# ConwayBeyond/Funscript-Flow

Measured on AMD Instinct MI355X. Metric: 1080p frame-pairs/sec, higher is better.
Workload: dtype f32

## Files before the change

### funscript_flow_amd/_capi.py

```python
import ctypes as C
import os
import sys

import numpy as np

_HERE = os.path.dirname(os.path.abspath(__file__))
LIB_PATH = os.path.join(_HERE, "csrc", "libffl_hip.so")

FFL_OK = 0
FFL_MAX_BATCH = 256
KERNEL_CLASSES = ["k_gray", "k_pyr_level", "k_polyexp", "k_frontend", "k_update_matrices", "k_blur_solve",
                  "k_pass1", "k_radial"]
FFL_PROFILE_ALL = 0xFF

FFL_MAX_CELLS = 64
CELL_DTYPE = np.dtype([(k, "<f8") for k in ("mean_u", "mean_v", "mean_mag", "var_mag")])
GRID_CENTRE_DTYPE = np.dtype([("cx", "<f8"), ("cy", "<f8"), ("total_var", "<f8"), ("cells", "<i4"), ("empty", "<i4")])
CENTERS = ("variance", "track")
FFL_MAX_TRACKS, FFL_MAX_TRACK_RADIUS = 8, 32
TRACK_ON_CUT = ("hold", "home")
TRACK_OK, TRACK_CUT, TRACK_LOST, TRACK_CLAMPED = 0, 1, 2, 4
TRACK_STATE_DTYPE = np.dtype([("x", "<f8"), ("y", "<f8"), ("home_x", "<f8"), ("home_y", "<f8"), ("steps", "<i8"),
                              ("lost_run", "<i4"), ("pad", "<i4")])
TRACK_DTYPE = np.dtype([("x", "<f8"), ("y", "<f8"), ("du", "<f8"), ("dv", "<f8"), ("sw", "<f8"), ("count", "<i4"), ("status", "<i4")])
# ... 605 lines not shown
    sw, sh = int(src_size[0]), int(src_size[1])
    win, b = (C.c_int * 4)(), C.c_size_t()
    code = layout if isinstance(layout, int) else yuv_layout(layout)
    info = source_info(rotate, mirror, yuv_range)
    geom = (int(resize[0]), int(resize[1]), int(crop[0]), int(crop[1]), int(out_size[0]), int(out_size[1]), win, C.byref(b))
    if depth == 8:
        rc = _src_call(load(), "ffl_frontend_yuv_window", info, sw, sh, code, int(sw if stride is None else stride), *geom)
    else:
        rc = _src_call(load(), "ffl_frontend_yuv16_window", info, sw, sh, code, int(2 * sw if stride is None else stride),
                       int(depth), *geom)
    _check(rc, exc=ValueError)
    return tuple(win), b.value


def _map_array(map, out_size, supersample):
    if supersample not in REMAP_SUPERSAMPLES or isinstance(supersample, bool):
        raise ValueError(f"supersample must be one of {REMAP_SUPERSAMPLES}, got {supersample!r}")
    m = np.asarray(map)
    want = (supersample * int(out_size[1]), supersample * int(out_size[0]), 2)
    if m.dtype != np.int32 or m.shape != want:
        raise ValueError(f"a source map for a {out_size[0]}x{out_size[1]} operand at supersample={supersample} is an int32 array of "
                         f"shape {want} holding (qx, qy) in 1/32 px, got {m.dtype} {m.shape}")
    return np.ascontiguousarray(m)


def remap_check(map, out_size, src_size, supersample=1, rotate=0, mirror=False, yuv_range="limited"):
    info = source_info(rotate, mirror, yuv_range)
    m = _map_array(map, out_size, supersample)
    up, st, valid = (C.c_int * 4)(), (C.c_int * 4)(), C.c_size_t()
    _check(load().ffl_remap_check(m.ctypes.data, int(out_size[0]), int(out_size[1]), int(supersample), int(src_size[0]),
                                  int(src_size[1]), C.byref(info) if info is not None else None, up, st, C.byref(valid)),
           exc=ValueError)
    return tuple(up), tuple(st), valid.value


def remap_bytes(out_size, supersample=1):
    return _sizes("ffl_remap_bytes", out_size[0], out_size[1], supersample)


class Remap:

    def __init__(self, id, src_size, supersample, window, valid):
        self.id, self.src_size, self.supersample, self.window, self.valid = id, tuple(src_size), supersample, window, valid

    def __repr__(self):
        return f"Remap(id={self.id}, src_size={self.src_size}, supersample={self.supersample}, window={self.window})"


_i, _u, _f, _pd, _sz, _u64, _vp, _str = C.c_int, C.c_uint, C.c_float, C.c_ssize_t, C.c_size_t, C.c_uint64, C.c_void_p, C.c_char_p
_ip, _i32p, _fp, _dp, _szp, _vpp = (C.POINTER(t) for t in (C.c_int, C.c_int32, C.c_float, C.c_double, C.c_size_t, C.c_void_p))
_P = C.POINTER
_ctx = _vp
_FRAMES = (_ctx, _i, _i, _vpp, _i, _i, _pd)
_DEVICE = (_ctx, _i, _i, _vp, _i)
_YUV_WIN = (_i, _i, _i, _pd)
_PAIRS = (_ctx, _i, _ip, _ip, _ip, _i)
_RADIAL = (_ctx, _i, _ip, _dp, _dp, _ip, _i, _dp)
_WINDOW = (_ctx, _i, _ip, _i, _i, _i, _f, _i)
_SRC = "_src"
SIGNATURES = {
    "ffl_device_count": (_i, ()),
    "ffl_create": (_i, (_i,) * 6 + (_vpp,)),
    "ffl_destroy": (None, (_ctx,)),
    "ffl_last_error": (_str, (_ctx,)),
    "ffl_device_mem_info": (_i, (_i, _szp, _szp)),
    "ffl_estimate_bytes": (_i, (_i,) * 5 + (_szp, _szp)),
    "ffl_upload_frame": (_i, (_ctx, _i, _vp, _i, _i, _i, _pd)),
    "ffl_upload_frames": (_i, (_ctx, _i, _i, _vpp, _i, _i, _i, _pd)),
    "ffl_upload_frames_raw": (_i, _FRAMES + (_i,) * 5),
    "ffl_upload_frames_raw_src": _SRC,
    "ffl_upload_frames_yuv": (_i, _FRAMES + (_i,) * 5),
    "ffl_frontend_yuv_window": (_i, _YUV_WIN + (_i,) * 6 + (_ip, _szp)),
    "ffl_upload_frames_yuv_src": _SRC,
    "ffl_frontend_yuv_window_src": _SRC,
    "ffl_upload_frames_yuv16": (_i, _FRAMES + (_i,) * 7),
    "ffl_frontend_yuv16_window": (_i, _YUV_WIN + (_i,) * 7 + (_ip, _szp)),
    "ffl_upload_frames_yuv16_src": _SRC,
    "ffl_frontend_yuv16_window_src": _SRC,
    "ffl_dev_frame_check": (_i, (_i,) * 3 + (_P(DevFrame),) + (_i,) * 6),
    "ffl_upload_frames_device": (_i, _DEVICE + (_i,) * 6 + (_u64,)),
    "ffl_dev_frame_check16": (_i, (_i,) * 4 + (_P(DevFrame),) + (_i,) * 6),
    "ffl_upload_frames_device16": (_i, _DEVICE + (_i,) * 8 + (_u64,)),
    "ffl_dev_frame_check_src": _SRC,
    "ffl_dev_frame_check16_src": _SRC,
    "ffl_upload_frames_device_src": _SRC,
    "ffl_upload_frames_device16_src": _SRC,
    "ffl_remap_check": (_i, (_vp,) + (_i,) * 5 + (_P(SourceInfo), _ip, _ip, _szp)),
    "ffl_remap_bytes": (_i, (_i,) * 3 + (_szp,)),
    "ffl_remap_create": (_i, (_ctx, _vp, _i, _i, _i, _ip)),
    "ffl_remap_destroy": (_i, (_ctx, _i)),
    "ffl_upload_frames_remap": (_i, (_ctx, _i, _i, _vpp, _i, _i, _i, _pd, _i, _i, _i, _P(SourceInfo))),
    "ffl_upload_frames_device_remap": (_i, _DEVICE + (_i,) * 5 + (_u64, _P(SourceInfo))),
    "ffl_export_flows": (_i, (_ctx, _i, _ip, _vp, _i, _pd, _u64)),
    "ffl_dev_flow_check": (_i, (_i,) * 4 + (_P(DevFlow),)),
    "ffl_import_flows": (_i, (_ctx, _i, _ip, _P(DevFlow), _i, _i, _u64)),
    "ffl_host_alloc": (_i, (_ctx, _sz, _vpp)),
    "ffl_host_free": (_i, (_ctx, _vp)),
    "ffl_flow_pairs": (_i, _PAIRS),
    "ffl_pass1_result": (_i, (_ctx, _i, _f, _i32p, _i32p, _fp, _fp, _ip)),
    "ffl_pass1_results": (_i, (_ctx, _i, _ip, _f, _i32p, _i32p, _fp, _fp, _ip)),
    "ffl_radial": (_i, _RADIAL),
    "ffl_radial_window": (_i, _WINDOW + (_vp, _u64)),
    "ffl_radial_axes": (_i, _RADIAL),
    "ffl_radial_window_axes": (_i, _WINDOW + (_vp, _u64)),
    "ffl_axes_extra_bytes": (_i, (_i, _i, _szp)),
    "ffl_dev_weights_check": (_i, (_i,) * 3 + (_P(DevWeights),)),
    "ffl_pass1_weighted": (_i, (_ctx, _i, _ip, _P(DevWeights), _i, _u64)),
    "ffl_radial_window_axes_weighted": (_i, _WINDOW + (_P(DevWeights), _vp, _u64)),
    "ffl_weights_extra_bytes": (_i, (_i, _i, _szp)),
    "ffl_consistency_default_params": (_i, (_P(ConsistencyParams),)),
    "ffl_consistency_params_check": (_i, (_P(ConsistencyParams),)),
    "ffl_consistency_weights": (_i, (_ctx, _i, _ip, _ip, _P(ConsistencyParams), _P(DevWeights), _P(DevWeights), _u64)),
    "ffl_residual_default_params": (_i, (_P(ResidualParams),)),
    "ffl_residual_params_check": (_i, (_P(ResidualParams),)),
    "ffl_residual_weights": (_i, (_ctx, _i, _ip, _ip, _ip, _P(ResidualParams), _P(DevWeights), _P(DevWeights), _u64)),
    "ffl_texture_default_params": (_i, (_P(TextureParams),)),
    "ffl_texture_params_check": (_i, (_P(TextureParams),)),
    "ffl_texture_weights": (_i, (_ctx, _i, _ip, _P(TextureParams), _P(DevWeights), _P(DevWeights), _u64)),
    "ffl_cell_grid_check": (_i, (_i,) * 3 + (_ip, _ip)),
    "ffl_cell_stats": (_i, (_ctx, _i, _ip, _i, _vp, _vp, _u64)),
    "ffl_radial_window_axes_centres": (_i, _WINDOW + (_vp, _pd, _vp, _u64)),
    "ffl_cells_extra_bytes": (_i, (_i,) * 3 + (_szp,)),
    "ffl_track_default_params": (_i, (_P(TrackParams),)),
    "ffl_track_params_check": (_i, (_P(TrackParams),)),
    "ffl_track_advance": (_i, (_ctx, _i, _ip, _i, _P(TrackParams), _P(DevWeights), _vp, _vp, _u64)),
    "ffl_roi_default_params": (_i, (_P(RoiParams),)),
    "ffl_roi_params_check": (_i, (_P(RoiParams),)),
    "ffl_roi_weights": (_i, (_ctx, _i, _vp, _pd, _P(RoiParams), _P(DevWeights), _P(DevWeights), _u64)),
    "ffl_radial_window_axes_weighted_centres": (_i, _WINDOW + (_P(DevWeights), _vp, _pd, _vp, _u64)),
    "ffl_motion_default_params": (_i, (_P(MotionParams),)),
    "ffl_motion_params_check": (_i, (_P(MotionParams),)),
    "ffl_motion_solve": (_i, (_dp, _i, _vp)),
    "ffl_motion_extra_bytes": (_i, (_i, _i, _szp)),
    "ffl_motion_fit": (_i, (_ctx, _i, _ip, _P(MotionParams), _P(DevWeights), _vp, _pd, _vp, _vp, _u64)),
    "ffl_motion_subtract": (_i, (_ctx, _i, _ip, _ip, _vp, _pd, _i, _u64)),
    "ffl_download_flow": (_i, (_ctx, _i, _vp)),
    "ffl_upload_flow": (_i, (_ctx, _i, _vp, _i)),
    "ffl_submit_pair": (_i, (_ctx, _i, _vp, _vp, _i, _i, _i, _pd, _i)),
    "ffl_sync": (_i, (_ctx,)),
    "ffl_dis_default_params": (_i, (_P(DisParams),)),
    "ffl_dis_geometry": (_i, (_i, _i, _P(DisParams), _ip, _ip)),
    "ffl_flow_pairs_dis": (_i, _PAIRS + (_P(DisParams),)),
    "ffl_debug_dis_pair": (_i, (_ctx, _i, _i, _P(DisParams), _i, _i, _vp)),
    "ffl_farneback_default_params": (_i, (_P(FarnebackParams),)),
    "ffl_farneback_geometry": (_i, (_i, _i, _P(FarnebackParams), _ip, _szp)),
    "ffl_farneback_extra_bytes": (_i, (_i,) * 3 + (_P(FarnebackParams), _szp)),
    "ffl_flow_pairs_farneback": (_i, _PAIRS + (_P(FarnebackParams),)),
    "ffl_flow_pairs_farneback_ex": (_i, _PAIRS + (_P(FarnebackParams), _u)),
    "ffl_num_levels": (_i, (_ctx,)),
    "ffl_level_size": (_i, (_ctx, _i, _ip)),
    "ffl_download_frame": (_i, (_ctx, _i, _vp)),
    "ffl_debug_pair": (_i, (_ctx,) + (_i,) * 4 + (_vp,) * 6),
    "ffl_debug_blur_plan": (_i, (_i,) * 9 + (_ip, _ip, _ip, _ip, _i)),
    "ffl_set_option": (_i, (_str, _i)),
    "ffl_ctx_set_option": (_i, (_ctx, _str, _i)),
    "ffl_ctx_get_option": (_i, (_ctx, _str, _ip)),
    "ffl_graph_stats": (_i, (_ctx, _ip, _ip, _ip)),
    "ffl_profile_enable": (_i, (_ctx, _u)),
    "ffl_profile_read": (_i, (_ctx, _i, _ip, _dp)),
    "ffl_kernel_name": (_str, (_i,)),
}
for _name, _sig in SIGNATURES.items():
    if _sig is _SRC:
        SIGNATURES[_name] = (SIGNATURES[_name[:-4]][0], SIGNATURES[_name[:-4]][1] + (_P(SourceInfo),))
EXPORTS = list(SIGNATURES)
RECORDS = {"ffl_source_info": SourceInfo, "ffl_dev_frame": DevFrame, "ffl_dev_flow": DevFlow, "ffl_pass2_record": PASS2_DTYPE,
           "ffl_axes_record": PASS2_AXES_DTYPE, "ffl_dev_weights": DevWeights, "ffl_consistency_params": ConsistencyParams,
           "ffl_residual_params": ResidualParams, "ffl_texture_params": TextureParams,
           "ffl_cell_record": CELL_DTYPE, "ffl_grid_centre": GRID_CENTRE_DTYPE, "ffl_motion_params": MotionParams,
           "ffl_motion_record": MOTION_DTYPE, "ffl_dis_params": DisParams, "ffl_track_params": TrackParams,
           "ffl_track_state": TRACK_STATE_DTYPE, "ffl_track_record": TRACK_DTYPE, "ffl_roi_params": RoiParams,
           "ffl_farneback_params": FarnebackParams}

_lib = None


def load():
    global _lib
    if _lib is not None:
        return _lib
    if not os.path.exists(LIB_PATH):
        raise FFLError(f"{LIB_PATH} is missing: build it with `make -C funscript_flow_amd/csrc` "
                       "(there is no CPU fallback for the HIP backend)")
    L = C.CDLL(LIB_PATH)
    for name, (restype, argtypes) in SIGNATURES.items():
        fn = getattr(L, name)
        fn.restype, fn.argtypes = restype, argtypes
    _lib = L
    return L


def set_option(name, value):
    if load().ffl_set_option(name.encode(), int(value)) != FFL_OK:
        raise FFLError(f"ffl_set_option({name!r}, {value}) rejected")


def get_option(name):
    v = C.c_int()
    if load().ffl_ctx_get_option(None, name.encode(), C.byref(v)) != FFL_OK:
        raise FFLError(f"unknown option {name!r}")
    return v.value


def blur_plan(tiles_x, tiles_y, n_pairs, slots, blur_rows=0, blur_min_wgs=3500, blur_taper=0, blur_taper_pairs=0,
              tile_order=0, blocks=True):
    L = load()
    args = [int(v) for v in (tiles_x, tiles_y, n_pairs, slots, blur_rows, blur_min_wgs, blur_taper, blur_taper_pairs, tile_order)]
    seg, n, grid = (C.c_int * 15)(), C.c_int(), C.c_int()
    _check(L.ffl_debug_blur_plan(*args, seg, C.byref(n), C.byref(grid), None, 0), exc=ValueError)
    segments = [tuple(seg[5 * i:5 * i + 5]) for i in range(n.value)]
    if not blocks:
        return segments, grid.value, None
    out = np.zeros((grid.value, 4), np.int32)
    _check(L.ffl_debug_blur_plan(*args, seg, C.byref(n), C.byref(grid), out.ctypes.data_as(_ip), grid.value), exc=ValueError)
    return segments, grid.value, out


def device_count():
    return load().ffl_device_count()


def device_mem_info(device=0):
    return _sizes("ffl_device_mem_info", device, outs=2)


def estimate_bytes(width, height, frame_slots, flow_slots, max_batch):
    return _sizes("ffl_estimate_bytes", width, height, frame_slots, flow_slots, max_batch, outs=2)


def axes_extra_bytes(width, height):
    return _sizes("ffl_axes_extra_bytes", width, height)


def weights_extra_bytes(width, height):
    return _sizes("ffl_weights_extra_bytes", width, height)


def cells_extra_bytes(width, height, cells):
    return _sizes("ffl_cells_extra_bytes", width, height, cells)


def motion_extra_bytes(width, height):
    return _sizes("ffl_motion_extra_bytes", width, height)


def cell_grid(width, height, cells):
    gw, gh = C.c_int(), C.c_int()
    _check(load().ffl_cell_grid_check(int(width), int(height), int(cells), C.byref(gw), C.byref(gh)))
    return gw.value, gh.value


def _centre_entries(centres, n_seq):
    if isinstance(centres, tuple) and len(centres) == 2 and isinstance(centres[1], (int, np.integer)):
        base, stride = centres
        return (int(base) if isinstance(base, (int, np.integer)) else _array_view(base)[0]), int(stride)
    ptr, shp, st, ts = _array_view(centres)
    if ts in ("<f8", "torch.float64") and len(shp) == 2:
        if shp != (n_seq, 2) or st[1] != 8:
            raise ValueError(f"centres: float64 shape {shp} with byte strides {st}, ({n_seq}, 2) with adjacent (cx, cy) is needed")
        return ptr, (st[0] if n_seq > 1 else 16)
    ptr, extent = _device_span(centres)
    if extent < n_seq * GRID_CENTRE_DTYPE.itemsize:
        raise ValueError(f"centres: {extent} bytes, {n_seq} centre records need {n_seq * GRID_CENTRE_DTYPE.itemsize}")
    return ptr, GRID_CENTRE_DTYPE.itemsize


def _iarr(v):
    a = np.ascontiguousarray(v, dtype=np.intc)
    return a.ctypes.data_as(C.POINTER(C.c_int)), a


def _darr(v):
    a = np.ascontiguousarray(v, dtype=np.float64)
    return a.ctypes.data_as(C.POINTER(C.c_double)), a


class Context:

    def __init__(self, width, height, device=0, frame_slots=None, flow_slots=None, max_batch=8):
        self.L = load()
        self.width, self.height, self.device, self.max_batch = int(width), int(height), int(device), int(max_batch)
        self.frame_slots = int(frame_slots if frame_slots is not None else 2 * max_batch + 2)
        self.flow_slots = int(flow_slots if flow_slots is not None else 13 + 2 * max_batch)
        h = C.c_void_p()
        rc = self.L.ffl_create(self.device, self.width, self.height, self.frame_slots, self.flow_slots, self.max_batch,
                               C.byref(h))
        if rc != FFL_OK:
            raise FFLError(f"ffl_create failed ({rc}): {self.L.ffl_last_error(None).decode()}")
        self._h = h

    def close(self):
        if getattr(self, "_h", None):
            self.L.ffl_destroy(self._h)
            self._h = None

    __del__ = close

    def __enter__(self):
        return self

    def __exit__(self, *a):
        self.close()

    def _chk(self, rc):
        if rc != FFL_OK:
            _check(rc, self._h)

    def upload_frame(self, fslot, frame):
        if frame.dtype != np.uint8 or frame.ndim not in (2, 3):
            raise FFLError("frame must be uint8 (H,W) or (H,W,3)")
        ch = 1 if frame.ndim == 2 else frame.shape[2]
        if frame.strides[-1] != 1 or (frame.ndim == 3 and frame.strides[1] != ch):
            frame = np.ascontiguousarray(frame)
        self._chk(self.L.ffl_upload_frame(self._h, fslot, frame.ctypes.data, frame.shape[1], frame.shape[0], ch,
                                          frame.strides[0]))

    def upload_frames(self, first_slot, frames):
        f0 = frames[0]
        shape, strides = f0.shape, f0.strides
        if f0.dtype == np.uint8 and f0.ndim in (2, 3) and strides[-1] == 1 and (f0.ndim == 2 or strides[1] == shape[2]):
            n = len(frames)
            ptrs = np.empty(n, np.uintp)
            uniform = True
            for i, f in enumerate(frames):
                if f.shape != shape or f.strides != strides or f.dtype != np.uint8:
                    uniform = False
                    break
                ptrs[i] = f.__array_interface__["data"][0]
            if uniform:
                ch = 1 if f0.ndim == 2 else shape[2]
                self._chk(self.L.ffl_upload_frames(self._h, first_slot, n, ptrs.ctypes.data_as(C.POINTER(C.c_void_p)), shape[1], shape[0],
                                                   ch, strides[0]))
                return
        fr = [f if (f.strides[-1] == 1 and (f.ndim == 2 or f.strides[1] == f.shape[2])) else np.ascontiguousarray(f)
              for f in frames]
        f0 = fr[0]
        ch = 1 if f0.ndim == 2 else f0.shape[2]
        if any(f.dtype != np.uint8 or f.shape != f0.shape or f.strides[0] != f0.strides[0] for f in fr):
            raise FFLError("upload_frames needs uint8 frames of one shape and row stride")
        ptrs = (C.c_void_p * len(fr))(*[f.ctypes.data for f in fr])
        self._chk(self.L.ffl_upload_frames(self._h, first_slot, len(fr), ptrs, f0.shape[1], f0.shape[0], ch,
                                           f0.strides[0]))

    def pinned_frames(self, n, channels=1, size=None, yuv=False, depth=8):
        w, h = size if size is not None else (self.width, self.height)
        shape = (n, h * 3 // 2, w) if yuv else (n, h, w) + ((channels,) if channels != 1 else ())
        dtype = np.uint8
        if depth != 8:
            if not yuv:
                raise FFLError("pinned_frames: depth applies to 4:2:0 frames (yuv=True)")
            dtype = np.uint16 if yuv_depth(depth)[0] > 8 else np.uint8
        nbytes = int(np.prod(shape)) * np.dtype(dtype).itemsize
        p = C.c_void_p()
        self._chk(self.L.ffl_host_alloc(self._h, nbytes, C.byref(p)))
        buf = (C.c_uint8 * nbytes).from_address(p.value)
        return np.frombuffer(buf, dtype).reshape(shape)

    def upload_frames_raw(self, first_slot, frames, resize, crop=(0, 0), rgb_order=False, rotate=0, mirror=False,
                          yuv_range="limited"):
        info = source_info(rotate, mirror, yuv_range)
        fr = [f if (f.ndim == 3 and f.strides[2] == 1 and f.strides[1] == 3) else np.ascontiguousarray(f) for f in frames]
        f0 = fr[0]
        if any(f.dtype != np.uint8 or f.ndim != 3 or f.shape != f0.shape or f.shape[2] != 3 or
               f.strides[0] != f0.strides[0] for f in fr):
            raise FFLError("upload_frames_raw needs (h, w, 3) uint8 frames of one shape and row stride")
        ptrs = (C.c_void_p * len(fr))(*[f.ctypes.data for f in fr])
        self._chk(_src_call(self.L, "ffl_upload_frames_raw", info, self._h, first_slot, len(fr), ptrs, f0.shape[1], f0.shape[0],
                            f0.strides[0], int(bool(rgb_order)), int(resize[0]), int(resize[1]), int(crop[0]), int(crop[1])))
# ... 456 lines not shown
```

### funscript_flow_amd/csrc/ffl_api.hip

```cpp
#include "../../include/ffl.h"
#include "ffl_kernels.h"

#include <math.h>
#include <stdarg.h>
#include <stdio.h>
#include <string.h>

#include <algorithm>
#include <condition_variable>
#include <mutex>
#include <string>
#include <thread>
#include <vector>

#define FFL_EV_RING 16
#define FFL_RAW_RING 4

template <class H, class Arg, hipError_t (*Free)(Arg)>
struct Owned {
    H h = H();
    Owned() = default;
    explicit Owned(H take) : h(take) {}
    Owned(Owned &&o) noexcept : h(o.release()) {}
    Owned &operator=(Owned &&o) noexcept { std::swap(h, o.h); return *this; }
// ... 262 lines not shown
};
typedef std::unique_lock<std::recursive_mutex> CtxLock;

static int set_err(ffl_ctx *c, int code, const char *fmt, ...) {
    char buf[512];
    va_list ap;
    va_start(ap, fmt);
    vsnprintf(buf, sizeof(buf), fmt, ap);
    va_end(ap);
    if (c) c->err = buf;
    else g_create_error = buf;
    return code;
}

#define HIPCHK_AS(c, what, call)                                                                          \
    do {                                                                                                  \
        hipError_t e_ = (call);                                                                           \
        if (e_ != hipSuccess)                                                                             \
            return set_err(c, FFL_ERR_HIP, "%s failed: %s (%s:%d)", what, hipGetErrorString(e_), __FILE__, \
                           __LINE__);                                                                     \
    } while (0)
#define HIPCHK(c, call) HIPCHK_AS(c, #call, call)
#define HIPCHK_ALLOC(c, fn, buf, ...) HIPCHK_AS(c, #fn "(" #buf ", " #__VA_ARGS__ ")", (buf).alloc(__VA_ARGS__))

static inline int cv_round(double v) { return (int)lrint(v); }

static void gaussian_kernel(int n, double sigma, float *out) {
    static const float tab1[] = {1.f};
    static const float tab3[] = {0.25f, 0.5f, 0.25f};
    static const float tab5[] = {0.0625f, 0.25f, 0.375f, 0.25f, 0.0625f};
    static const float tab7[] = {0.03125f, 0.109375f, 0.21875f, 0.28125f, 0.21875f, 0.109375f, 0.03125f};
    const float *fixed = nullptr;
    if (sigma <= 0 && (n & 1) && n <= 7) fixed = n == 1 ? tab1 : n == 3 ? tab3 : n == 5 ? tab5 : tab7;
    double sg = sigma > 0 ? sigma : ((n - 1) * 0.5 - 1) * 0.3 + 0.8;
    double scale2x = -0.5 / (sg * sg);
    double sum = 0;
    for (int i = 0; i < n; i++) {
        double x = i - (n - 1) * 0.5;
        double t = fixed ? (double)fixed[i] : exp(scale2x * x * x);
        out[i] = (float)t;
        sum += out[i];
    }
    sum = 1.0 / sum;
    for (int i = 0; i < n; i++) out[i] = (float)(out[i] * sum);
}

static void farneback_prepare_gaussian(int n, double sigma, FbgPoly *out) {
    float gg[2 * 7 + 1];
    double s = 0;
    for (int x = -n; x <= n; x++) {
        gg[x + n] = (float)exp(-x * x / (2 * sigma * sigma));
        s += gg[x + n];
    }
    s = 1. / s;
    for (int x = -n; x <= n; x++) gg[x + n] = (float)(gg[x + n] * s);
    for (int x = 0; x <= n; x++) {
        out->g[x] = gg[x + n];
        out->xg[x] = (float)(x * gg[x + n]);
        out->xxg[x] = (float)(x * x * gg[x + n]);
    }
    double G[6][6];
    memset(G, 0, sizeof(G));
    for (int y = -n; y <= n; y++)
        for (int x = -n; x <= n; x++) {
            float p = gg[y + n] * gg[x + n];
            G[0][0] += p;
            G[1][1] += p * x * x;
            G[3][3] += p * x * x * x * x;
            G[5][5] += p * x * x * y * y;
        }
    G[2][2] = G[0][3] = G[0][4] = G[3][0] = G[4][0] = G[1][1];
    G[4][4] = G[3][3];
    G[3][4] = G[4][3] = G[5][5];
    double A[6][12];
    for (int i = 0; i < 6; i++)
        for (int j = 0; j < 12; j++) A[i][j] = j < 6 ? G[i][j] : (j - 6 == i ? 1.0 : 0.0);
    for (int c = 0; c < 6; c++) {
        int p = c;
        for (int r = c + 1; r < 6; r++)
            if (fabs(A[r][c]) > fabs(A[p][c])) p = r;
        if (p != c)
            for (int j = 0; j < 12; j++) { double t = A[c][j]; A[c][j] = A[p][j]; A[p][j] = t; }
        double d = 1.0 / A[c][c];
        for (int j = 0; j < 12; j++) A[c][j] *= d;
        for (int r = 0; r < 6; r++)
            if (r != c) {
                double f = A[r][c];
                if (f != 0)
                    for (int j = 0; j < 12; j++) A[r][j] -= f * A[c][j];
            }
    }
    out->ig11 = A[1][7];
    out->ig03 = A[0][9];
    out->ig33 = A[3][9];
    out->ig55 = A[5][11];
}

static void polyexp_prepare(PolyConsts *pc) {
    FbgPoly q;
    farneback_prepare_gaussian(FFL_POLY_N, 1.2, &q);
    for (int x = 0; x <= FFL_POLY_N; x++) {
        pc->g[x] = q.g[x];
        pc->xg[x] = q.xg[x];
        pc->xxg[x] = q.xxg[x];
        pc->gd[x] = (double)pc->g[x];
        pc->xxgd[x] = (double)pc->xxg[x];
    }
    pc->ig11 = q.ig11;
    pc->ig03 = q.ig03;
    pc->ig33 = q.ig33;
    pc->ig55 = q.ig55;
}

struct LevelRule {
    int levels;
    int lw[FBG_MAX_SCALES], lh[FBG_MAX_SCALES], ksize[FBG_MAX_SCALES];
    double sigma[FBG_MAX_SCALES];
};
static void level_rule(int w, int h, double pyr_scale, int levels, LevelRule *r) {
    int k;
    double scale = 1.0;
    for (k = 0; k < levels; k++) {
        scale *= pyr_scale;
        if (w * scale < 32 || h * scale < 32) break;
    }
    r->levels = k;
    for (k = 0; k <= r->levels; k++) {
        double sc = 1.0;
        for (int i = 0; i < k; i++) sc *= pyr_scale;
        r->sigma[k] = (1.0 / sc - 1.0) * 0.5;
        const int sm = cv_round(r->sigma[k] * 5) | 1;
        r->ksize[k] = sm < 3 ? 3 : sm;
        r->lw[k] = cv_round(w * sc);
        r->lh[k] = cv_round(h * sc);
    }
}

static void level_geometry(int w, int h, Geometry *geo) {
    LevelRule r;
    level_rule(w, h, 0.5, 3, &r);
    geo->levels = r.levels;
    for (int k = 0; k <= r.levels; k++) {
        LevelGeom &g = geo->lv[k];
        g.lw = r.lw[k];
        g.lh = r.lh[k];
        g.ksize = r.ksize[k];
        g.sigma = r.sigma[k];
        memset(&g.gk, 0, sizeof(g.gk));
        g.gk.ksize = g.ksize;
        gaussian_kernel(g.ksize, g.sigma, g.gk.k);
    }
}

#define FFL_FRAME_SIZE_RULE "unsupported frame size %dx%d (16x16 .. 20*w*h < 2^32)"
static bool frame_size_ok(int w, int h) { return !(w < 16 || h < 16 || (long)w * h * 20 >= (1L << 32)); }
static bool counts_ok(int n_frame_slots, int n_flow_slots, int max_batch) {
    return n_frame_slots >= 2 && n_flow_slots >= 1 && max_batch >= 1 && max_batch <= FFL_MAX_BATCH;
}

static Layout context_layout(int w, int h, int n_frame_slots, int n_flow_slots, int max_batch) {
    Geometry geo;
    level_geometry(w, h, &geo);
    const size_t N = (size_t)w * h, maxU = 2 * (size_t)max_batch;
    Layout l = {};
    for (int k = 0; k <= geo.levels; k++) {
        const size_t plane = (size_t)geo.lv[k].lw * geo.lv[k].lh;
        l.i_off[k] = l.I; l.t_off[k] = l.T; l.r_off[k] = l.R;
        l.I += plane * maxU;
        l.T += ffl_pyr_tmp_floats(w, h, geo.lv[k].lw) * maxU;
        l.R += 5 * plane * maxU;
    }
    l.M = 5 * N * max_batch; l.flow = 2 * N * max_batch;
    l.p1 = (size_t)ffl_pass1_blocks(w, h) * max_batch; l.tab = FFL_EV_RING;
    l.gray = (size_t)n_frame_slots * N; l.bgr = (size_t)n_frame_slots * N * 3;
    l.slots = 2 * N * n_flow_slots; l.res = n_flow_slots;
    return l;
}

static hipEvent_t prof_event(ffl_ctx *c) {
    Event e;
    if (c->prof_pool.empty()) {
        hipEventCreate(e.put());
    } else {
        e = std::move(c->prof_pool.back());
        c->prof_pool.pop_back();
    }
    return e.release();
}

struct ProfScope {
    ffl_ctx *c;
    int cls;
    hipEvent_t a = nullptr, b = nullptr;
    bool on, shared = false;
    ProfScope(ffl_ctx *c_, int cls_, hipStream_t st, bool chain = false)
        : c(c_), cls(cls_), on((c_->prof_mask >> cls_) & 1u) {
        if (on) {
            stream = st;
            if (chain && c->prof_last_end && c->prof_last_cls == cls && c->prof_last_stream == st) {
                a = c->prof_last_end;
                shared = true;
            } else {
                a = prof_event(c);
                hipEventRecord(a, st);
            }
        } else {
            c->prof_last_end = nullptr;
        }
    }
    ~ProfScope() {
        if (on) {
            b = prof_event(c);
            hipEventRecord(b, stream);
            c->prof_recs.push_back({cls, a, b, shared});
            c->prof_last_end = b;
            c->prof_last_cls = cls;
            c->prof_last_stream = stream;
        }
    }
    hipStream_t stream = nullptr;
};

static void prof_collect(ffl_ctx *c) {
    for (auto &r : c->prof_recs) {
        float ms = 0;
        hipEventSynchronize(r.b);
        hipEventElapsedTime(&ms, r.a, r.b);
        c->prof_launches[r.cls]++;
        c->prof_ms[r.cls] += ms;
    }
    for (auto &r : c->prof_recs) {
        if (!r.shared_start) c->prof_pool.emplace_back(r.a);
        c->prof_pool.emplace_back(r.b);
    }
    c->prof_recs.clear();
    c->prof_last_end = nullptr;
}

struct WaitOnce {
    hipStream_t st;
    hipEvent_t seen[8];
    int n = 0;
    explicit WaitOnce(hipStream_t s) : st(s) {}
    hipError_t operator()(hipEvent_t e) {
        if (!e) return hipSuccess;
        for (int k = 0; k < n; k++)
            if (seen[k] == e) return hipSuccess;
        if (n < 8) seen[n++] = e;
        return hipStreamWaitEvent(st, e, 0);
    }
};

static int wait_unlocked(ffl_ctx *c, CtxLock &lk, const hipEvent_t *evs, int n) {
    HIPCHK(c, hipSetDevice(c->device));
    lk.unlock();
    hipError_t e = hipSuccess;
    for (int i = 0; i < n && e == hipSuccess; i++)
        if (evs[i]) e = hipEventSynchronize(evs[i]);
    lk.lock();
    if (e != hipSuccess) return set_err(c, FFL_ERR_HIP, "hipEventSynchronize failed: %s", hipGetErrorString(e));
    return FFL_OK;
}

static int wait_frame_free(ffl_ctx *c, WaitOnce &wait_copy, int fs) {
    const size_t nl = c->frame_readers();
    for (size_t l = 0; l < nl; l++) HIPCHK(c, wait_copy(c->ev_last_use[(size_t)fs * nl + l].get()));
    return FFL_OK;
}

static int publish_frames(ffl_ctx *c, int first, int n) {
    EvRef ev;
    HIPCHK(c, c->up_ring.record(c->s_copy, &ev));
    for (int i = first; i < first + n; i++) {
        c->ev_uploaded[i] = ev;
        c->frame_valid[i] = 1;
    }
    return FFL_OK;
}

static void publish_slots(ffl_ctx *c, int n, const int *slots, EvRef done, bool ready) {
    for (int i = 0; i < n; i++) {
        c->ev_slot_done[slots[i]] = done;
        c->slot_state[slots[i]] = ready;
    }
}

static int check_frame_run(ffl_ctx *c, const char *fn, int first, int n, const void *table, const uint8_t *const *frames = nullptr) {
    if (!table || n < 1 || first < 0 || first + n > c->n_fslots)
        return set_err(c, FFL_ERR_INVALID, "%s: bad frame slot range %d..%d", fn, first, first + n - 1);
    for (int i = 0; frames && i < n; i++)
        if (!frames[i]) return set_err(c, FFL_ERR_INVALID, "%s: frame %d is NULL", fn, i);
    return FFL_OK;
}

static bool flow_slot_ok(const ffl_ctx *c, int slot) { return slot >= 0 && slot < c->n_slots; }
static int check_flow_slots(ffl_ctx *c, const char *fn, int n, const int *slots, const char *holds, const char *repeat_rule) {
    for (int i = 0; i < n; i++) {
        if (!flow_slot_ok(c, slots[i])) return set_err(c, FFL_ERR_INVALID, "%s: flow slot %d out of range", fn, slots[i]);
        if (holds && !c->slot_state[slots[i]]) return set_err(c, FFL_ERR_STATE, "%s: flow slot %d holds no %s", fn, slots[i], holds);
    }
    if (!repeat_rule) return FFL_OK;
    int dup = -1;
    for (int i = 0; i < n; i++) {
        if (c->slot_mark[slots[i]] && dup < 0) dup = slots[i];
        c->slot_mark[slots[i]] = 1;
    }
// ... 561 lines not shown
                           crop_x, crop_y, out_w, out_h, win, bytes);
}

int ffl_frontend_yuv16_window_src(int src_w, int src_h, int layout, ptrdiff_t stride_bytes, int depth, int resize_w, int resize_h,
                                  int crop_x, int crop_y, int out_w, int out_h, int win[4], size_t *bytes,
                                  const ffl_source_info *si) {
    return frontend_window("ffl_frontend_yuv16_window", src_w, src_h, layout, stride_bytes, 2, depth, si, resize_w, resize_h,
                           crop_x, crop_y, out_w, out_h, win, bytes);
}

static int send_yuv(ffl_ctx *c, CtxLock &lk, const char *fn, int first, int n, const uint8_t *const *frames, int sw, int sh,
                    ptrdiff_t stride_bytes, int layout, int es, int depth, int msb, FrontParams &fp, const YuvWin &yw,
                    const RemapParams *rp) {
    for (int i = 0; es == 2 && i < n; i++)
        if ((uintptr_t)frames[i] & 1) return set_err(c, FFL_ERR_INVALID, "%s: frame %d is not 2-byte aligned", fn, i);
    HIPCHK(c, hipSetDevice(c->device));
    fp.kind = es == 2 ? FFL_SRC_YUV16 : FFL_SRC_YUV;
    fp.rgb = 0;
    if (es == 2) front_depth(&fp, depth, msb);
    const bool nv12 = layout == FFL_YUV_NV12;
    const size_t ybytes = (size_t)yw.w * yw.h * es, fbytes = ybytes * 3 / 2;
    struct Plane {
        size_t src, dst;
        ptrdiff_t pitch;
        size_t row;
        int rows;
    } pl[3];
    const size_t cw = (size_t)sw / 2 * es, ch = (size_t)sh / 2;
    const size_t wrow = (size_t)yw.w * es, x0 = (size_t)yw.x0 * es;
    pl[0] = {(size_t)yw.y0 * stride_bytes + x0, 0, stride_bytes, wrow, yw.h};
    int np = 3;
    if (nv12) {
        pl[1] = {(size_t)(sh + yw.y0 / 2) * stride_bytes + x0, ybytes, stride_bytes, wrow, yw.h / 2};
        np = 2;
    } else {
        const size_t u0 = (size_t)sh * sw * es + (size_t)(yw.y0 / 2) * cw + x0 / 2;
        pl[1] = {u0, ybytes, (ptrdiff_t)cw, wrow / 2, yw.h / 2};
        pl[2] = {u0 + ch * cw, ybytes + ybytes / 4, (ptrdiff_t)cw, wrow / 2, yw.h / 2};
    }
    const size_t span = (size_t)stride_bytes * (sh + sh / 2 - 1) + (size_t)sw * es;
    auto direct = [&](int i) {
        bool ok = in_host_buf(c, frames[i], span);
        for (int k = 0; ok && k < np; k++) ok = ((uintptr_t)(frames[i] + pl[k].src) | (size_t)pl[k].pitch | pl[k].row) % 4 == 0;
        return ok;
    };
    auto stage = [&](int i, uint8_t *h, int threads) {
        const uint8_t *src[2] = {frames[i] + pl[0].src, nullptr};
        c->pool.copy(h, src, 1, pl[0].pitch, pl[0].row, pl[0].rows, threads);
        src[0] = frames[i] + pl[1].src;
        if (!nv12) src[1] = frames[i] + pl[2].src;
        c->pool.copy(h + pl[1].dst, src, nv12 ? 1 : 2, pl[1].pitch, pl[1].row, pl[1].rows, threads);
    };
    auto send_direct = [&](int i, uint8_t *d) -> int {
        for (int k = 0; k < np; k++)
            HIPCHK(c, hipMemcpy2DAsync(d + pl[k].dst, pl[k].row, frames[i] + pl[k].src, (size_t)pl[k].pitch, pl[k].row,
                                       (size_t)pl[k].rows, hipMemcpyHostToDevice, c->s_copy));
        return FFL_OK;
    };
    auto desc = [&](const uint8_t *d) {
        FrameDesc s = {};
        s.p0 = d;
        s.p1 = d + ybytes;
        s.p2 = nv12 ? s.p1 + es : s.p1 + ybytes / 4;
        s.pitch0 = wrow;
        s.pitch1 = s.pitch2 = nv12 ? wrow : wrow / 2;
        s.c_step = (nv12 ? 2 : 1) * es;
        s.wx = yw.x0;
        s.wy = yw.y0;
        return s;
    };
    return upload_staged(c, lk, first, n, fbytes, fp, direct, stage, send_direct, desc, rp);
}

static int upload_yuv(ffl_ctx *c, const char *fn, int first, int n, const uint8_t *const *frames, int sw, int sh,
                      ptrdiff_t stride_bytes, int layout, int es, int depth, int msb, int rw, int rh, int crop_x, int crop_y,
                      const ffl_source_info *si) {
    if (!c) return FFL_ERR_INVALID;
    std::unique_lock<std::mutex> ul(c->up_mu);
    CtxLock lk(c->mu);
    if (int rc = check_frame_run(c, fn, first, n, frames, frames)) return rc;
    FrontParams fp;
    YuvWin yw;
    if (int rc = yuv_window(c, fn, sw, sh, layout, stride_bytes, es, depth, si, rw, rh, crop_x, crop_y, c->w, c->h, &fp, &yw))
        return rc;
    return send_yuv(c, lk, fn, first, n, frames, sw, sh, stride_bytes, layout, es, depth, msb, fp, yw, nullptr);
}

int ffl_upload_frames_yuv(ffl_ctx *c, int first, int n, const uint8_t *const *frames, int sw, int sh, ptrdiff_t stride_bytes,
                          int layout, int rw, int rh, int crop_x, int crop_y) {
    return upload_yuv(c, "ffl_upload_frames_yuv", first, n, frames, sw, sh, stride_bytes, layout, 1, 8, 0, rw, rh, crop_x, crop_y,
                      nullptr);
}

int ffl_upload_frames_yuv_src(ffl_ctx *c, int first, int n, const uint8_t *const *frames, int sw, int sh, ptrdiff_t stride_bytes,
                              int layout, int rw, int rh, int crop_x, int crop_y, const ffl_source_info *si) {
    return upload_yuv(c, "ffl_upload_frames_yuv", first, n, frames, sw, sh, stride_bytes, layout, 1, 8, 0, rw, rh, crop_x, crop_y, si);
}

int ffl_upload_frames_yuv16(ffl_ctx *c, int first, int n, const uint16_t *const *frames, int sw, int sh, ptrdiff_t stride_bytes,
                            int layout, int depth, int msb_aligned, int rw, int rh, int crop_x, int crop_y) {
    return upload_yuv(c, "ffl_upload_frames_yuv16", first, n, (const uint8_t *const *)frames, sw, sh, stride_bytes, layout, 2,
                      depth, msb_aligned != 0, rw, rh, crop_x, crop_y, nullptr);
}

int ffl_upload_frames_yuv16_src(ffl_ctx *c, int first, int n, const uint16_t *const *frames, int sw, int sh, ptrdiff_t stride_bytes,
                                int layout, int depth, int msb_aligned, int rw, int rh, int crop_x, int crop_y,
                                const ffl_source_info *si) {
    return upload_yuv(c, "ffl_upload_frames_yuv16", first, n, (const uint8_t *const *)frames, sw, sh, stride_bytes, layout, 2,
                      depth, msb_aligned != 0, rw, rh, crop_x, crop_y, si);
}

int ffl_upload_frame(ffl_ctx *c, int fslot, const uint8_t *data, int width, int height, int channels,
                     ptrdiff_t stride_bytes) {
    return ffl_upload_frames(c, fslot, 1, &data, width, height, channels, stride_bytes);
}

int ffl_download_frame(ffl_ctx *c, int fslot, uint8_t *dst) {
    if (!c) return FFL_ERR_INVALID;
    CtxLock lk(c->mu);
    if (!dst || fslot < 0 || fslot >= c->n_fslots)
        return set_err(c, FFL_ERR_INVALID, "ffl_download_frame: bad frame slot %d", fslot);
    if (!c->frame_valid[fslot]) return set_err(c, FFL_ERR_STATE, "ffl_download_frame: frame slot %d was never uploaded", fslot);
    HIPCHK(c, hipSetDevice(c->device));
    HIPCHK(c, hipMemcpyAsync(dst, c->d_gray + (size_t)fslot * c->N, c->N, hipMemcpyDeviceToHost, c->s_copy));
    HIPCHK(c, hipStreamSynchronize(c->s_copy));
    return FFL_OK;
}

struct DebugCapture {
    int level, iter;
    float *I0, *I1, *R0, *R1, *M, *flow;
};

static int enqueue_batch(ffl_ctx *c, ffl_ctx::Lane &L, const BatchTab &T, int n, int nU, int pov_mode, const DebugCapture *cap) {
    hipStream_t st = L.st;
    const size_t N = c->N;
    const UTab *ut = &L.d_tab->ut;
    const PairTab *pt = &L.d_tab->pt;
    const PyrJob *l0 = &L.pyr[L.n_jobs - 1];
    const bool fuse_l0 = c->opt.fuse_l0_blur && ffl_polyexp_from_gray_ok(*l0);
    const int skip_l0 = fuse_l0 && !cap;
    {
        ProfScope ps(c, FFL_K_PYRAMID, st);
        if (!ffl_launch_pyr_multi(c->d_gray, N, ut, nU, L.pyr, L.n_jobs - skip_l0, c->opt, st))
            for (int k = c->geo.levels; k >= skip_l0; k--)
                ffl_launch_pyr_level(c->d_gray, N, ut, nU, L.pyr[c->geo.levels - k], st);
    }
    {
        ProfScope ps(c, FFL_K_POLYEXP, st);
        ffl_launch_polyexp_multi(L.poly, L.n_jobs, nU, c->pc, c->d_gray, N, ut, fuse_l0 ? l0 : nullptr, st);
    }

    int pw = 0, ph = 0;
    for (int k = c->geo.levels; k >= 0; k--) {
        const LevelGeom &g = c->geo.lv[k];
        const int lw = g.lw, lh = g.lh;
        const size_t plane = (size_t)lw * lh;
        const size_t I_stride = plane, R_stride = 5 * plane, M_stride = 5 * plane;
        float *Rk = L.d_R + c->lay.r_off[k];
        if (pw == 0 && cap)
            for (int i = 0; i < n; i++) HIPCHK(c, hipMemsetAsync(T.pt.flow[k][i], 0, sizeof(float) * 2 * plane, st));
        int mi = 0;
        const bool fuse_first = c->opt.fuse_first > 0 && !cap && (long)((lw + 63) / 64) * ((lh + 15) / 16) * n >= c->opt.fuse_first;
        if (!fuse_first) {
            ProfScope ps(c, FFL_K_UPDATE_MATRICES, st);
            ffl_launch_update_matrices(Rk, R_stride, plane, pt, k, n, L.d_M[mi], M_stride, lw, lh, pw, ph, pw == 0, cap != nullptr, c->opt, st);
        }
        bool captured = false;
        auto capture = [&]() -> int {
            HIPCHK(c, hipStreamSynchronize(st));
            if (cap->I0) HIPCHK(c, hipMemcpy(cap->I0, L.d_I + c->lay.i_off[k] + (size_t)T.pt.u0[0] * I_stride, sizeof(float) * plane, hipMemcpyDeviceToHost));
            if (cap->I1) HIPCHK(c, hipMemcpy(cap->I1, L.d_I + c->lay.i_off[k] + (size_t)T.pt.u1[0] * I_stride, sizeof(float) * plane, hipMemcpyDeviceToHost));
            if (cap->R0) HIPCHK(c, hipMemcpy(cap->R0, Rk + (size_t)T.pt.u0[0] * R_stride, sizeof(float) * 5 * plane, hipMemcpyDeviceToHost));
            if (cap->R1) HIPCHK(c, hipMemcpy(cap->R1, Rk + (size_t)T.pt.u1[0] * R_stride, sizeof(float) * 5 * plane, hipMemcpyDeviceToHost));
            if (cap->M) HIPCHK(c, hipMemcpy(cap->M, L.d_M[mi], sizeof(float) * 5 * plane, hipMemcpyDeviceToHost));
            if (cap->flow) HIPCHK(c, hipMemcpy(cap->flow, T.pt.flow[k][0], sizeof(float) * 2 * plane, hipMemcpyDeviceToHost));
            captured = true;
            return FFL_OK;
        };
        for (int it = 0; it < 3; it++) {
            if (cap && cap->level == k && cap->iter == it) {
                int rc = capture();
                if (rc) return rc;
            }
            const int update = it < 2;
            {
                ProfScope ps(c, FFL_K_BLUR_SOLVE, st, it > 0 && !cap);
                if (it == 0 && fuse_first)
                    ffl_launch_blur_solve_first(L.d_M[mi ^ 1], M_stride, Rk, R_stride, plane, pt, k, n, lw, lh, pw, ph, c->opt, c->blur_slots, st);
                else
                    ffl_launch_blur_solve(L.d_M[mi], L.d_M[mi ^ 1], M_stride, Rk, R_stride, plane, pt, k, n, lw, lh,
                                          update, cap != nullptr, c->opt, c->blur_slots, st);
            }
            if (update) mi ^= 1;
        }
        if (cap && cap->level == k && !captured) {
            int rc = capture();
            if (rc) return rc;
        }
        pw = lw;
        ph = lh;
    }
    {
        ProfScope ps(c, FFL_K_PASS1, st);
        ffl_launch_pass1(pt, n, c->w, c->h, pov_mode, L.d_pkey, L.d_psum, st);
    }
    return FFL_OK;
}

static int batch_graph(ffl_ctx *c, ffl_ctx::Lane &L, const BatchTab &T, int n, int nU, int pov_mode,
                       ffl_ctx::Lane::GraphEntry **ge) {
    *ge = nullptr;
    for (auto &g : L.graphs)
        if (g.n == n && g.nU == nU && g.pov == pov_mode && g.epoch == c->opt_epoch) *ge = &g;
    if (*ge || c->graph_bad_epoch == c->opt_epoch) return FFL_OK;
    hipStream_t st = L.st;
    ffl_ctx::Lane::GraphEntry g = {n, nU, pov_mode, c->opt_epoch, Graph(), GraphExec()};
    hipError_t fail = hipStreamBeginCapture(st, hipStreamCaptureModeThreadLocal);
    if (fail == hipSuccess) {
        const int rc = enqueue_batch(c, L, T, n, nU, pov_mode, nullptr);
        fail = hipStreamEndCapture(st, g.graph.put());
        if (fail == hipSuccess && (rc != FFL_OK || !g.graph)) fail = hipErrorStreamCaptureInvalidated;
        if (fail == hipSuccess) fail = hipGraphInstantiate(g.exec.put(), g.graph, nullptr, nullptr, 0);
    }
    if (fail != hipSuccess) {
        g.exec.reset();
        g.graph.reset();
        (void)hipGetLastError();
        c->graph_bad_epoch = c->opt_epoch;
        c->graph_failed++;
        if (!c->graph_fail_reported) {
            c->graph_fail_reported = true;
            fprintf(stderr, "libffl_hip: hipGraph capture of a %d-pair batch failed (%s); this context launches its batches "
                            "one kernel at a time until its options change (results are unaffected)\n", n, hipGetErrorString(fail));
        }
        return FFL_OK;
    }
    if (L.graphs.size() >= 16) {
        HIPCHK(c, hipStreamSynchronize(st));
        L.graphs.erase(L.graphs.begin());
    }
    L.graphs.push_back(std::move(g));
    *ge = &L.graphs.back();
    c->graph_captured++;
    return FFL_OK;
}

static int fbg_work(ffl_ctx *c, ffl_ctx::Lane &L, const FbgPlan &p, int nU, FbgWork *wk);

static int queue_batch(ffl_ctx *c, ffl_ctx::Lane &L, BatchTab &T, int *nU_out, int n, const int *f0, const int *f1,
                       const int *slots, int pov_mode, const DebugCapture *cap, const DisKParams *dis,
                       const FbgPlan *fbg) {
    hipStream_t st = L.st;
    const size_t N = c->N;
    int nU = 0;
    auto uidx = [&](int fs) {
        int &u = c->u_of_fslot[fs];
        if (u < 0) {
            T.ut.fslot[nU] = fs;
            u = nU++;
        }
        return u;
    };
    for (int i = 0; i < n; i++) {
        T.pt.u0[i] = uidx(f0[i]);
        T.pt.u1[i] = uidx(f1[i]);
        T.pt.res[i] = c->d_res + slots[i];
    }
    for (int k = c->geo.levels; k >= 0; k--) {
        const size_t plane = (size_t)c->geo.lv[k].lw * c->geo.lv[k].lh;
        float *buf = ((c->geo.levels - k) & 1) ? L.d_flowB : L.d_flowA;
        for (int i = 0; i < n; i++)
            T.pt.flow[k][i] = (k == 0) ? c->d_flow + (size_t)slots[i] * 2 * N : buf + (size_t)i * 2 * plane;
    }
    for (int k = c->geo.levels + 1; k < FFL_MAX_LEVELS; k++)
        for (int i = 0; i < n; i++) T.pt.flow[k][i] = nullptr;
    for (int i = 0; i < nU; i++) c->u_of_fslot[T.ut.fslot[i]] = -1;
    *nU_out = nU;
    WaitOnce wait(st);
    for (int i = 0; i < nU; i++) HIPCHK(c, wait(c->ev_uploaded[T.ut.fslot[i]].get()));
    for (int i = 0; i < n; i++) HIPCHK(c, wait(c->ev_slot_done[slots[i]].get()));
    HIPCHK(c, hipMemcpyAsync(L.d_tab, &T, sizeof(BatchTab), hipMemcpyHostToDevice, st));

    if (fbg || dis) {
        if (fbg) {
            FbgWork wk;
            if (int rc = fbg_work(c, L, *fbg, nU, &wk)) return rc;
            ffl_launch_fb_general(&L.d_tab->ut, &L.d_tab->pt, n, nU, c->d_gray, N, c->w, c->h, *fbg, wk, st);
        } else {
            ffl_launch_dis(&L.d_tab->ut, &L.d_tab->pt, n, c->d_gray, N, L.d_M[0], *dis, st);
        }
        ProfScope ps(c, FFL_K_PASS1, st);
        ffl_launch_pass1(&L.d_tab->pt, n, c->w, c->h, pov_mode, L.d_pkey, L.d_psum, st);
    } else if (c->opt.use_graph && !cap && c->prof_mask == 0) {
        ffl_ctx::Lane::GraphEntry *ge;
        if (int rc = batch_graph(c, L, T, n, nU, pov_mode, &ge)) return rc;
        if (ge) {
            HIPCHK(c, hipGraphLaunch(ge->exec, st));
            c->graph_replayed++;
        } else if (int rc = enqueue_batch(c, L, T, n, nU, pov_mode, nullptr)) {
            return rc;
        }
    } else if (int rc = enqueue_batch(c, L, T, n, nU, pov_mode, cap)) {
        return rc;
    }
    HIPCHK(c, hipGetLastError());
    return FFL_OK;
// ... 1764 lines not shown
    *mode = (ps == 2 * e && cs == e && (e == 4 || al4)) ? FFL_IMP_NHWC : (e == 4 && ps == 4) ? FFL_IMP_NCHW : FFL_IMP_ANY;
    return FFL_OK;
}

int ffl_dev_flow_check(int dtype, int n, int width, int height, const ffl_dev_flow *f) {
    int mode;
    size_t bytes;
    return dev_flow_check(nullptr, "ffl_dev_flow_check", dtype, n, width, height, f, &mode, &bytes);
}

int ffl_import_flows(ffl_ctx *c, int n, const int *slots, const ffl_dev_flow *f, int dtype, int pov_mode, uint64_t stream) {
    static const char *fn = "ffl_import_flows";
    if (!c) return FFL_ERR_INVALID;
    std::unique_lock<std::mutex> pl(c->post_mu);
    CtxLock lk(c->mu);
    ExportTab t;
    if (int rc = open_slot_list(c, fn, "fields", n, slots, nullptr, &t)) return rc;
    int mode;
    size_t bytes;
    if (int rc = dev_flow_check(c, fn, dtype, n, c->w, c->h, f, &mode, &bytes)) return rc;
    hipStream_t cst;
    const PostRegion reg{"the flow fields", f->base, bytes, "host flow fields go through ffl_upload_flow"};
    if (int rc = post_begin(c, fn, stream, &cst, &reg, 1, n, slots)) return rc;
    const ImportArgs a{(const char *)f->base, (long long)f->item_stride, (long long)f->row_pitch, (long long)f->pixel_stride,
                       (long long)f->channel_stride, c->d_flow, c->d_res};
    {
        ProfScope ps(c, FFL_K_PASS1, c->s_post);
        ffl_launch_import_pass1(a, t, n, dtype, mode, c->w, c->h, pov_mode ? 1 : 0, c->d_ptab, c->d_pskey, c->d_rpsum,
                                c->s_post);
    }
    return post_end(c, cst, n, slots);
}

int ffl_upload_flow(ffl_ctx *c, int slot, const float *src, int pov_mode) {
    if (!c) return FFL_ERR_INVALID;
    std::unique_lock<std::mutex> pl(c->post_mu);
    CtxLock lk(c->mu);
    if (!flow_slot_ok(c, slot) || !src) return set_err(c, FFL_ERR_INVALID, "ffl_upload_flow: bad arguments");
    hipStream_t st = c->s_post;
    hipEvent_t ev = c->ev_slot_done[slot].get();
    if (int rc = wait_unlocked(c, lk, &ev, 1)) return rc;
    lk.unlock();
    hipError_t se = hipStreamSynchronize(st);
    lk.lock();
    HIPCHK(c, se);
    HIPCHK(c, hipMemcpy(c->d_flow + (size_t)slot * 2 * c->N, src, sizeof(float) * 2 * c->N, hipMemcpyHostToDevice));
    c->h_ptab->flow[0][0] = c->d_flow + (size_t)slot * 2 * c->N;
    c->h_ptab->res[0] = c->d_res + slot;
    HIPCHK(c, hipMemcpyAsync(c->d_ptab, c->h_ptab, sizeof(PairTab), hipMemcpyHostToDevice, st));
    {
        ProfScope ps(c, FFL_K_PASS1, st);
        ffl_launch_pass1(c->d_ptab, 1, c->w, c->h, pov_mode, c->d_pskey, c->d_rpsum, st);
    }
    EvRef done;
    if (int rc = publish_post(c, 1, &slot, &done)) return rc;
    HIPCHK(c, hipGetLastError());
    return FFL_OK;
}

int ffl_submit_pair(ffl_ctx *c, int slot, const uint8_t *prev, const uint8_t *next, int width, int height, int channels,
                    ptrdiff_t stride_bytes, int pov_mode) {
    if (!c) return FFL_ERR_INVALID;
    if (!flow_slot_ok(c, slot) || 2 * slot + 1 >= c->n_fslots) {
        CtxLock lk(c->mu);
        return set_err(c, FFL_ERR_INVALID, "ffl_submit_pair: slot %d needs frame slots %d,%d and a flow slot", slot, 2 * slot, 2 * slot + 1);
    }
    int rc = ffl_upload_frame(c, 2 * slot, prev, width, height, channels, stride_bytes);
    if (rc) return rc;
    rc = ffl_upload_frame(c, 2 * slot + 1, next, width, height, channels, stride_bytes);
    if (rc) return rc;
    int f0 = 2 * slot, f1 = 2 * slot + 1;
    return ffl_flow_pairs(c, 1, &f0, &f1, &slot, pov_mode);
}

int ffl_sync(ffl_ctx *c) {
    if (!c) return FFL_ERR_INVALID;
    std::unique_lock<std::mutex> ul(c->up_mu);
    std::unique_lock<std::mutex> pl(c->post_mu);
    CtxLock lk(c->mu);
    std::vector<hipEvent_t> evs;
    evs.push_back(ev_latest(c->up_ring).get());
    for (auto &rb : c->raw)
        if (rb.busy) evs.push_back(rb.ev);
    for (auto &L : c->lanes) evs.push_back(ev_latest(L.ring).get());
    evs.push_back(ev_latest(c->post_ring).get());
    pl.unlock();
    ul.unlock();
    return wait_unlocked(c, lk, evs.data(), (int)evs.size());
}

static constexpr struct { const char *name; int value; } kFixedKnobs[] = {
    {"blur_tile_h", 16}, {"run_ahead", 0}, {"merge_expand", 1}};
static const int *fixed_knob(const char *name) {
    for (const auto &k : kFixedKnobs)
        if (!strcmp(name, k.name)) return &k.value;
    return nullptr;
}
static const FflOptionRow *option_row(const char *name) {
    for (const FflOptionRow &r : kFflOptionRows)
        if (!strcmp(name, r.name)) return &r;
    return nullptr;
}

static int set_option_impl(FflOptions &o, const char *name, int value, bool live) {
    if (const int *fixed = fixed_knob(name)) return value == *fixed ? FFL_OK : FFL_ERR_INVALID;
    const FflOptionRow *r = option_row(name);
    if (!r || value < r->lo || value > r->hi) return FFL_ERR_INVALID;
    if (live && r->member == &FflOptions::lanes) return value == o.lanes ? FFL_OK : FFL_ERR_STATE;
    o.*r->member = r->flag ? value != 0 : value;
    return FFL_OK;
}

static int get_option_impl(const FflOptions &o, const char *name, int *value) {
    const int *fixed = fixed_knob(name);
    const FflOptionRow *r = option_row(name);
    if (!fixed && !r) return FFL_ERR_INVALID;
    *value = fixed ? *fixed : o.*r->member;
    return FFL_OK;
}

int ffl_debug_blur_plan(int tiles_x, int tiles_y, int n_pairs, int slots, int blur_rows, int blur_min_wgs, int blur_taper,
                        int blur_taper_pairs, int tile_order, int *segments, int *n_segments, int *grid, int *blocks,
                        int max_blocks) {
    FflOptions o;
    if (tiles_x < 1 || tiles_y < 1 || n_pairs < 1 || n_pairs > FFL_MAXB || slots < 0 || !segments || !n_segments || !grid ||
        set_option_impl(o, "blur_rows", blur_rows, false) || set_option_impl(o, "blur_min_wgs", blur_min_wgs, false) ||
        set_option_impl(o, "blur_taper", blur_taper, false) || set_option_impl(o, "blur_taper_pairs", blur_taper_pairs, false) ||
        set_option_impl(o, "tile_order", tile_order, false))
        return set_err(nullptr, FFL_ERR_INVALID, "ffl_debug_blur_plan: bad size, pair count, slot count, option value or NULL output");
    BlurPlan plan;
    const unsigned g = ffl_blur_plan(tiles_x, tiles_y, n_pairs, slots, o, &plan);
    *n_segments = plan.n;
    *grid = (int)g;
    for (int i = 0; i < FFL_BLUR_SEGS; i++) {
        const BlurSeg &s = plan.s[i];
        const int row[5] = {s.first_block, s.first_pair, s.pairs, s.nrb, s.strips};
        memcpy(segments + 5 * i, row, sizeof(row));
    }
    if (!blocks) return FFL_OK;
    if ((unsigned)max_blocks < g)
        return set_err(nullptr, FFL_ERR_INVALID, "ffl_debug_blur_plan: %u workgroups, room for %d", g, max_blocks);
    for (unsigned blk = 0; blk < g; blk++) {
        int b, tile_x, row0, nrb;
        int *out = blocks + 4 * (size_t)blk;
        if (ffl_blur_block(plan, blk, tiles_x, tile_order, b, tile_x, row0, nrb)) {
            out[0] = b; out[1] = tile_x; out[2] = row0; out[3] = std::max(0, std::min(nrb, tiles_y - row0));
        } else {
            out[0] = -1; out[1] = out[2] = out[3] = 0;
        }
    }
    return FFL_OK;
}

int ffl_set_option(const char *name, int value) {
    if (!name) return FFL_ERR_INVALID;
    std::lock_guard<std::mutex> g(g_opt_mu);
    return set_option_impl(g_opts, name, value, false);
}

int ffl_ctx_set_option(ffl_ctx *c, const char *name, int value) {
    if (!c || !name) return FFL_ERR_INVALID;
    CtxLock lk(c->mu);
    const int rc = set_option_impl(c->opt, name, value, true);
    if (rc == FFL_OK) c->opt_epoch++;
    else if (rc == FFL_ERR_STATE) set_err(c, rc, "ffl_ctx_set_option: \"lanes\" is fixed once the context exists (%d)", c->opt.lanes);
    else set_err(c, rc, "ffl_ctx_set_option: unknown option or value out of range: %s = %d", name, value);
    return rc;
}

int ffl_ctx_get_option(ffl_ctx *c, const char *name, int *value) {
    if (!name || !value) return FFL_ERR_INVALID;
    if (!c) {
        std::lock_guard<std::mutex> g(g_opt_mu);
        return get_option_impl(g_opts, name, value);
    }
    CtxLock lk(c->mu);
    return get_option_impl(c->opt, name, value);
}

int ffl_graph_stats(ffl_ctx *c, int *captured, int *replayed, int *capture_failures) {
    if (!c) return FFL_ERR_INVALID;
    CtxLock lk(c->mu);
    if (captured) *captured = c->graph_captured;
    if (replayed) *replayed = c->graph_replayed;
    if (capture_failures) *capture_failures = c->graph_failed;
    return FFL_OK;
}

int ffl_profile_enable(ffl_ctx *c, unsigned class_mask) {
    if (!c) return FFL_ERR_INVALID;
    int rc = ffl_sync(c);
    if (rc) return rc;
    CtxLock lk(c->mu);
    prof_collect(c);
    c->prof_mask = class_mask;
    return FFL_OK;
}

int ffl_profile_read(ffl_ctx *c, int k, int *launches, double *total_ms) {
    if (!c || k < 0 || k >= FFL_K_COUNT) return FFL_ERR_INVALID;
    int rc = ffl_sync(c);
    if (rc) return rc;
    CtxLock lk(c->mu);
    prof_collect(c);
    if (launches) *launches = c->prof_launches[k];
    if (total_ms) *total_ms = c->prof_ms[k];
    c->prof_launches[k] = 0;
    c->prof_ms[k] = 0;
    return FFL_OK;
}

}
```

### funscript_flow_amd/csrc/ffl_kernels.h

```cpp
#pragma once
#include <hip/hip_runtime.h>
#include <limits.h>
#include <stdint.h>

#define FFL_MAXB 256
#define FFL_MAXU (2 * FFL_MAXB)
#define FFL_MAX_LEVELS 4
#define FFL_POLY_N 5
#define FFL_WIN 15
#define FFL_WIN_R 7

struct PolyConsts {
    float g[FFL_POLY_N + 1], xg[FFL_POLY_N + 1], xxg[FFL_POLY_N + 1];
    double gd[FFL_POLY_N + 1], xxgd[FFL_POLY_N + 1];
    double ig11, ig03, ig33, ig55;
};

struct GaussKernel {
    float k[32];
    int ksize;
};

struct UTab {
    int fslot[FFL_MAXU];
};

struct PairTab {
    int u0[FFL_MAXB], u1[FFL_MAXB];
    float *flow[FFL_MAX_LEVELS][FFL_MAXB];
    struct Pass1Result *res[FFL_MAXB];
};

struct BatchTab {
    UTab ut;
    PairTab pt;
};

struct Pass1Result {
    int x, y;
    float div_val;
    int weighted;
    double mag_sum;
};
__host__ __device__ inline double ffl_record_mean(const Pass1Result &r, double npx) {
    return r.weighted ? r.mag_sum : r.mag_sum / npx;
}

enum { FFL_FRONT_GENERIC = 0, FFL_FRONT_AREA2 = 1, FFL_FRONT_IDENTITY = 2 };
enum { FFL_SRC_GRAY = 0, FFL_SRC_BGR = 1, FFL_SRC_YUV = 2, FFL_SRC_YUV16 = 3, FFL_SRC_ANY = -1 };
struct FrameDesc {
    const uint8_t *p0, *p1, *p2;
    long long pitch0, pitch1, pitch2;
    long long ps, cs;
    int c_step;
    int wx, wy;
    int fslot;
};
struct FrontParams {
    int kind, rgb;
    int sw, sh;
    int cx, cy, ow, oh;
    double scale_x, scale_y;
    int mode;
    int shift16, round16;
    int src;
    int ax, bx, cx0, ay, by, cy0;
    int full;
};
#define FFL_REMAP_NONE (-2147483647 - 1)
struct RemapParams {
    const int2 *map;
    int ss, lg;
};
struct ExportTab {
    int slot[FFL_MAXB];
};

enum { FFL_IMP_F32 = 0, FFL_IMP_F16 = 1, FFL_IMP_BF16 = 2 };
enum { FFL_IMP_ANY = 0,
       FFL_IMP_NHWC = 1,
       FFL_IMP_NCHW = 2 };
struct ImportArgs {
    const char *base;
    long long item, pitch, ps, cs;
    float *flow;
    Pass1Result *res;
};

struct WeightArgs {
    const char *base;
    long long item, pitch;
};

#define FFL_MAX_JOBS 4
enum { FFL_PYR_NONE = -1, FFL_PYR_F1 = 0, FFL_PYR_F2, FFL_PYR_H4, FFL_PYR_H9, FFL_PYR_V4, FFL_PYR_V9, FFL_PYR_H1 };
struct PyrJob {
    int kind, w, h, lw, lh;
    unsigned gx, gy, first, count;
    double sx, sy;
    float *tmp, *I;
    size_t tmp_stride, I_stride;
    GaussKernel gk;
};
struct PyrJobs {
    PyrJob j[FFL_MAX_JOBS];
    int n;
};
struct PolyJob {
    const float *I;
    float *R;
    size_t I_stride, R_stride, plane;
    int w, h;
    unsigned gx, gy, first, count;
    int from_gray;
    float gk0, gk1;
};
struct PolyJobs {
    PolyJob j[FFL_MAX_JOBS];
    int n;
};

struct FflOptions {
    int lanes = 2;
    int fuse_first = 10000;
    int use_graph = 1;
    int copy_threads = 4;
    int blur_rows = 0;
    int blur_min_wgs = 3500;
    int tile_order = 0;
    int blur_taper = 1;
    int blur_taper_pairs = 0;
    int pyr_coarse = 1;
    int fuse_l0_blur = 1;
    int fb_general = 0;
};
struct FflOptionRow {
    const char *name;
    int FflOptions::*member;
    int lo, hi;
    bool flag;
};
inline constexpr FflOptionRow kFflOptionRows[] = {
    {"lanes", &FflOptions::lanes, 1, 4, false},
    {"fuse_first", &FflOptions::fuse_first, 0, INT_MAX, false},
    {"graph", &FflOptions::use_graph, INT_MIN, INT_MAX, true},
    {"copy_threads", &FflOptions::copy_threads, 1, 16, false},
    {"blur_rows", &FflOptions::blur_rows, 0, 64, false},
    {"blur_min_wgs", &FflOptions::blur_min_wgs, 1, INT_MAX, false},
    {"tile_order", &FflOptions::tile_order, 0, 1, false},
    {"blur_taper", &FflOptions::blur_taper, 0, 1, false},
    {"blur_taper_pairs", &FflOptions::blur_taper_pairs, 0, FFL_MAXB, false},
    {"pyr_coarse", &FflOptions::pyr_coarse, INT_MIN, INT_MAX, true},
    {"fuse_l0_blur", &FflOptions::fuse_l0_blur, INT_MIN, INT_MAX, true},
    {"fb_general", &FflOptions::fb_general, 0, 1, false},
};

#define FFL_BLUR_SEGS 3
struct BlurSeg {
    int first_block, first_pair, pairs, nrb, strips;
};
struct BlurPlan {
    BlurSeg s[FFL_BLUR_SEGS];
    int n;
};
struct BlurSlots {
    int first, first_zero, update, last;
};

bool ffl_launch_pyr_multi(const uint8_t *gray_base, size_t gray_stride, const UTab *ut, int nU, const PyrJob *levels, int n,
                          const FflOptions &opt, hipStream_t st);
bool ffl_polyexp_from_gray_ok(const PyrJob &l0);
void ffl_launch_polyexp_multi(const PolyJob *levels, int n, int nU, PolyConsts pc, const uint8_t *gray_base, size_t gray_stride,
                              const UTab *ut, const PyrJob *l0, hipStream_t st);
void ffl_launch_frontend(const FrameDesc &d, uint8_t *gray, const FrontParams &p, hipStream_t st);
void ffl_launch_frontend_dev(const FrameDesc *tab, int n, uint8_t *gray_base, size_t N, const FrontParams &p, hipStream_t st);
void ffl_launch_frontend_remap(const FrameDesc &d, uint8_t *gray, const FrontParams &p, const RemapParams &r, hipStream_t st);
void ffl_launch_frontend_remap_dev(const FrameDesc *tab, int n, uint8_t *gray_base, size_t N, const FrontParams &p,
                                   const RemapParams &r, hipStream_t st);
void ffl_launch_export_flows(const float *flow, const ExportTab &tab, int n, size_t N, char *dst, long long item_stride,
                             int layout, hipStream_t st);
void ffl_launch_import_pass1(const ImportArgs &a, const ExportTab &tab, int n, int dtype, int mode, int w, int h, int pov_mode,
                             PairTab *pt, unsigned long long *pkey, double *psum, hipStream_t st);
void ffl_launch_gray(const uint8_t *bgr, uint8_t *gray, int n_pixels, hipStream_t st);
size_t ffl_pyr_tmp_floats(int w, int h, int lw);
bool ffl_pyr_level_ok(int w, int h, int lw, int lh, int ksize);
void ffl_launch_pyr_level(const uint8_t *gray_base, size_t gray_stride, const UTab *ut, int nU, const PyrJob &level,
                          hipStream_t st);
void ffl_launch_update_matrices(const float *R, size_t R_stride, size_t plane, const PairTab *pt, int level, int nB, float *M,
                                size_t M_stride, int lw, int lh, int pw, int ph, int zero_flow, int store_flow,
                                const FflOptions &opt, hipStream_t st);
void ffl_launch_blur_solve(const float *Min, float *Mout, size_t M_stride, const float *R, size_t R_stride,
                           size_t plane, const PairTab *pt, int level, int nB, int lw, int lh, int update, int store_flow,
                           const FflOptions &opt, const BlurSlots &slots, hipStream_t st);


void ffl_launch_blur_solve_first(float *Mout, size_t M_stride, const float *R, size_t R_stride, size_t plane,
                                 const PairTab *pt, int level, int nB, int lw, int lh, int pw, int ph, const FflOptions &opt,
                                 const BlurSlots &slots, hipStream_t st);
bool ffl_blur_slots(BlurSlots *out);
unsigned ffl_blur_plan(int tiles_x, int tiles_y, int nB, int slots, const FflOptions &opt, BlurPlan *plan);

#define DIS_MAX_PATCHES 4096
#define DIS_MAX_SCALES 12
struct DisKParams {
    int w, h, finest, coarsest, stride, gd_iters, vr_iters, mean_norm, spatial_prop, stripes;
    float alpha, gamma, delta;
    size_t pair_floats;
    size_t pyr_floats;
    size_t pyr_off[DIS_MAX_SCALES];
    float *dbg;
    int dbg_scale, dbg_stage;
};
void ffl_launch_dis(const UTab *ut, const PairTab *pt, int nB, const uint8_t *gray, size_t gray_stride, float *scratch,
                    const DisKParams &p, hipStream_t st);

int ffl_pass1_blocks(int w, int h);
void ffl_launch_pass1(const PairTab *pt, int nB, int w, int h, int pov_mode, unsigned long long *pkey, double *psum,
                      hipStream_t st);

#define FFL_WINDOW_MAX_RADIUS 32
struct WindowSeq {
    int slot[FFL_MAXB + 2 * FFL_WINDOW_MAX_RADIUS];
};
struct WindowItem {
    const float *flow;
    double cx, cy;
    int cut, pad;
};
struct Pass2Record {
    double dot, cx, cy;
    float mean_mag, div_val;
    int x, y, cut, pad;
};
struct AxesRecord {
    Pass2Record base;
    double tangential, shift_x, shift_y, reserved;
};
#define FFL_NAXES 4
int ffl_radial_blocks(int w, int h);
struct RadialForm {
    int nc;
    const WeightArgs *maps;
};
void ffl_launch_radial(const WindowItem *tab, int n, int w, int h, int pov_mode, const double *wytab, const RadialForm &form,
                       double *psum, void *out, hipStream_t st);
void ffl_launch_pass1_weighted(const WeightArgs &wa, float *flow, Pass1Result *res, const ExportTab &tab, int n, int w, int h,
                               int pov_mode, PairTab *pt, unsigned long long *pkey, double *psum, double *psw, hipStream_t st);
void ffl_launch_window_plan(const WindowSeq &seq, int n_seq, int first, int n, int radius, float cut_threshold,
                            const Pass1Result *res, const float *flow, int w, int h, const void *cen, long long cstride,
                            WindowItem *tab, void *out, int rec_stride, hipStream_t st);

#define FFL_CELLS_MAX 64
struct CellRecord {
    double mean_u, mean_v, mean_mag, var_mag;
};
struct GridCentre {
    double cx, cy, total_var;
    int cells, empty;
};
void ffl_launch_cell_stats(const float *flow, const ExportTab &tab, int n, int w, int h, int G, CellRecord *cells,
                           GridCentre *centres, double *rowsum, hipStream_t st);

void ffl_launch_consistency(const float *flow, const ExportTab &fwd, const ExportTab &bwd, int n, int w, int h, float alpha,
                            float beta, int soft, const WeightArgs *gate, char *out, long long out_item, long long out_pitch,
                            hipStream_t st);

void ffl_launch_residual(const unsigned char *gray, const float *flow, const ExportTab &fr0, const ExportTab &fr1, const ExportTab &fl,
                         int n, int w, int h, float alpha, float beta, int soft, const WeightArgs *gate, char *out,
                         long long out_item, long long out_pitch, hipStream_t st);

void ffl_launch_texture(const unsigned char *gray, const ExportTab &fr, int n, int w, int h, int radius, float tau, int soft,
                        const WeightArgs *gate, char *out, long long out_item, long long out_pitch, hipStream_t st);

#define FFL_TRACK_MAX_R 32
#define FFL_TRACK_MAX_T 8
enum { TRK_HOLD = 0, TRK_HOME = 1 };
enum { TRK_OK = 0, TRK_CUT = 1, TRK_LOST = 2, TRK_CLAMPED = 4 };
struct TrackState {
    double x, y, home_x, home_y;
    long long steps;
    int lost_run, pad;
};
struct TrackRecord {
    double x, y, du, dv, sw;
    int count, status;
};
void ffl_launch_track(const float *flow, const Pass1Result *res, const ExportTab &tab, int n, int n_tracks, int w, int h,
                      int radius, int on_cut, float cut_threshold, const WeightArgs *maps, TrackState *state, TrackRecord *out,
                      hipStream_t st);
void ffl_launch_roi_weights(const char *cen, long long cstride, int n, int w, int h, float ax, float ay, int soft,
                            const WeightArgs *gate, char *out, long long out_item, long long out_pitch, hipStream_t st);

#define FFL_MOTION_NSUMS 12
enum { MOT_S = 0, MOT_SX, MOT_SY, MOT_SXX, MOT_SXY, MOT_SYY, MOT_SU, MOT_SUX, MOT_SUY, MOT_SV, MOT_SVX, MOT_SVY };
enum { MOT_TRANSLATION = 0, MOT_RIGID = 1, MOT_SIMILARITY = 2, MOT_AFFINE = 3 };
enum { MOT_OK = 0, MOT_EMPTY = 1, MOT_DEGENERATE = 2 };
struct MotionRecord {
    double a0, a1, a2, b0, b1, b2;
    double sw;
    int model, status;
};
struct MotionPrior {
    const char *base;
    long long stride;
};

__host__ __device__ inline void ffl_motion_solve_body(const double *s, int model, MotionRecord *out) {
    const double S = s[MOT_S], Sx = s[MOT_SX], Sy = s[MOT_SY], Sxx = s[MOT_SXX], Sxy = s[MOT_SXY], Syy = s[MOT_SYY];
    const double Su = s[MOT_SU], Sux = s[MOT_SUX], Suy = s[MOT_SUY], Sv = s[MOT_SV], Svx = s[MOT_SVX], Svy = s[MOT_SVY];
    MotionRecord r;
    r.a0 = r.a1 = r.a2 = r.b0 = r.b1 = r.b2 = 0.0;
    r.sw = S;
    r.model = model;
    r.status = MOT_EMPTY;
    if (S == 0.0) {
        *out = r;
        return;
    }
    const double ta = Su / S, tb = Sv / S;
    r.a0 = ta;
    r.b0 = tb;
    r.status = MOT_OK;
    const double eps = 1e-12;
    if (model == MOT_RIGID || model == MOT_SIMILARITY) {
        const double Q = Sxx + Syy;
        const double q = Sx / S, p = Sy / S;
        const double D = (Q - q * Sx) - p * Sy;
        if (!(S > eps * S) || !(D > eps * Q)) {
            r.status = MOT_DEGENERATE;
        } else {
            const double g3 = Svx - Suy;
            const double z3 = (g3 + p * Su) - q * Sv;
            const double rot = z3 / D;
            double sc = 0.0;
            if (model == MOT_SIMILARITY) {
                const double g2 = Sux + Svy;
                const double z2 = (g2 - q * Su) - p * Sv;
                sc = z2 / D;
            }
            r.a0 = (ta - q * sc) + p * rot;
            r.b0 = (tb - p * sc) - q * rot;
            r.a1 = sc;
            r.a2 = -rot;
            r.b1 = rot;
            r.b2 = sc;
        }
    } else if (model == MOT_AFFINE) {
        bool ok = S > eps * S;
        double l10 = 0.0, l20 = 0.0, l21 = 0.0, d1 = 0.0, d2 = 0.0;
        if (ok) {
            l10 = Sx / S;
// ... 225 lines not shown
```

### funscript_flow_amd/csrc/kernels_farneback.hip

```cpp
#include "ffl_kernels.h"

#include <algorithm>

__global__ __launch_bounds__(256) void k_gray(const uint8_t *__restrict__ bgr, uint8_t *__restrict__ gray, int n) {
    int i4 = (blockIdx.x * 256 + threadIdx.x) * 4;
    if (i4 + 3 < n) {
        const uint32_t *p = reinterpret_cast<const uint32_t *>(bgr + (size_t)i4 * 3);
        uint32_t a = p[0], b = p[1], c = p[2];
        uint32_t px[12] = {a & 255, (a >> 8) & 255, (a >> 16) & 255, a >> 24, b & 255, (b >> 8) & 255,
                           (b >> 16) & 255, b >> 24, c & 255, (c >> 8) & 255, (c >> 16) & 255, c >> 24};
        uint32_t o = 0;
#pragma unroll
        for (int j = 0; j < 4; j++) {
            uint32_t g = (px[j * 3] * 3735u + px[j * 3 + 1] * 19235u + px[j * 3 + 2] * 9798u + 16384u) >> 15;
            o |= g << (8 * j);
        }
        *reinterpret_cast<uint32_t *>(gray + i4) = o;
    } else {
        for (int i = i4; i < n; i++) {
            uint32_t b = bgr[(size_t)i * 3], g = bgr[(size_t)i * 3 + 1], r = bgr[(size_t)i * 3 + 2];
            gray[i] = (uint8_t)((b * 3735u + g * 19235u + r * 9798u + 16384u) >> 15);
        }
    }
}
// ... 783 lines not shown
        ffl_um_finish(cur.r0, bb, cur.inside, w, h, x, y, cur.f.x, cur.f.y, m);
        if (in) {
#pragma unroll
            for (int c = 0; c < 5; c++) *ffl_at<float>(M + c * plane, o) = m[c];
        }
        if (k + 1 < NR) cur = nxt;
    }
}

template <int MODE>
__global__ __launch_bounds__(256) void k_update_matrices(const float *__restrict__ R, size_t R_stride, size_t plane,
                                                         const PairTab *__restrict__ pt, int level,
                                                         float *__restrict__ M, size_t M_stride, int w,
                                                         int h, int pw, int ph, double usx, double usy, int store_flow,
                                                         int nB, int order) {
    int b, tile_x, tile_y;
    if (!ffl_tile_coord((w + 63) / 64, (h + 15) / 16, nB, order, b, tile_x, tile_y)) return;
    const int lx = threadIdx.x & 63, x0 = tile_x * 64, x = min(x0 + lx, w - 1);
    const bool xin = x0 + lx < w;
    const float *R0 = R + (size_t)pt->u0[b] * R_stride, *R1 = R + (size_t)pt->u1[b] * R_stride;
    float *flow = pt->flow[level][b];
    const float *pf = pt->flow[min(level + 1, FFL_MAX_LEVELS - 1)][b];
    constexpr int NR = 4;
    const int ybase = tile_y * 16 + (threadIdx.x >> 6);
    float2 f[NR];
    if (MODE == 1) {
        const bool half_scale = usx == 0.5 && usy == 0.5;
        int xa0, xa1;
        float a1;
        if (half_scale) ffl_resize_coord_half(x, pw, xa0, xa1, a1);
        else ffl_resize_coord(x, pw, usx, xa0, xa1, a1);
        const int xq = min(xa0, pw - 2);
        float4 c0[NR], c1[NR];
        float b1[NR];
#pragma unroll
        for (int k = 0; k < NR; k++) {
            int ya0, ya1;
            const int y = min(ybase + 4 * k, h - 1);
            if (half_scale) ffl_resize_coord_half(y, ph, ya0, ya1, b1[k]);
            else ffl_resize_coord(y, ph, usy, ya0, ya1, b1[k]);
            c0[k] = ffl_gload4(pf, 8u * ((unsigned)ya0 * (unsigned)pw + xq));
            c1[k] = ffl_gload4(pf, 8u * ((unsigned)ya1 * (unsigned)pw + xq));
        }
#pragma unroll
        for (int k = 0; k < NR; k++) f[k] = ffl_upsample2(c0[k], c1[k], xa0 == xq, xa1 == xq, a1, b1[k]);
    } else if (MODE == 0) {
#pragma unroll
        for (int k = 0; k < NR; k++) {
            const unsigned o = (unsigned)min(ybase + 4 * k, h - 1) * (unsigned)w + (unsigned)x;
            const FFL_GLOBAL float *q = (const FFL_GLOBAL float *)flow + 2u * o;
            f[k] = make_float2(q[0], q[1]);
        }
    } else {
#pragma unroll
        for (int k = 0; k < NR; k++) f[k] = make_float2(0.f, 0.f);
    }
    ffl_um_rows<NR>(R0, R1, M + (size_t)b * M_stride, plane, w, h, x, xin, ybase, [&](int k) { return f[k]; },
                    [&](unsigned o, float2 d) {
                        if (MODE == 1 && store_flow) {
                            flow[2u * o] = d.x;
                            flow[2u * o + 1u] = d.y;
                        }
                    });
}

void ffl_launch_update_matrices(const float *R, size_t R_stride, size_t plane, const PairTab *pt, int level, int nB,
                                float *M,
                                size_t M_stride, int lw, int lh, int pw, int ph, int zero_flow, int store_flow,
                                const FflOptions &opt, hipStream_t st) {
    dim3 grid(ffl_tile_grid((lw + 63) / 64, (lh + 15) / 16, nB));
    const auto k = pw > 0 ? k_update_matrices<1> : (zero_flow ? k_update_matrices<2> : k_update_matrices<0>);
    hipLaunchKernelGGL(k, grid, dim3(256), 0, st, R, R_stride, plane, pt, level, M, M_stride, lw, lh, pw, ph,
                       pw > 0 ? (double)pw / lw : 1.0, pw > 0 ? (double)ph / lh : 1.0, pw > 0 ? store_flow : 0, nB,
                       opt.tile_order);
}

#ifndef FFL_K5_WAVES
#define FFL_K5_WAVES 4
#endif
#ifndef FFL_K5_WAVES_FIRST
#define FFL_K5_WAVES_FIRST 3
#endif
#ifndef FFL_K5_GROUP_FIRST
#define FFL_K5_GROUP_FIRST 3
#endif
#ifndef FFL_K5_GROUP
#define FFL_K5_GROUP 3
#endif

__device__ __forceinline__ void ffl_box_block16(const float (&v)[30], double (&out)[16]) {
    double s[15];
    s[14] = (double)v[14];
#pragma unroll
    for (int j = 13; j >= 0; j--) s[j] = (double)v[j] + s[j + 1];
    double p = (double)v[15];
    out[0] = s[0];
#pragma unroll
    for (int t = 1; t < 15; t++) {
        out[t] = s[t] + p;
        p = p + (double)v[15 + t];
    }
    out[15] = p;
}

template <int Q>
__device__ __forceinline__ void ffl_box_quarter(const double (&d)[18], double (&out)[4]) {
    constexpr int NA = 15 - 4 * Q;
    double S[4] = {0.0, 0.0, 0.0, 0.0};
    double s = d[NA - 1];
    if (NA - 1 < 4) S[NA - 1] = s;
#pragma unroll
    for (int j = NA - 2; j >= 0; j--) {
        s = d[j] + s;
        if (j < 4) S[j] = s;
    }
    double p = d[NA];
#pragma unroll
    for (int m = 0; m <= 4 * Q + 2; m++) {
        if (m > 0) p = p + d[NA + m];
        const int i = m + 1 - 4 * Q;
        if (i >= 0 && i < 4) {
            if (4 * Q + i == 15) out[i] = p;
            else out[i] = S[i] + p;
        }
    }
    if (Q == 0) out[0] = S[0];
}

#ifdef FFL_STAMP
#define FFL_NSTAMP 16
__device__ unsigned long long g_stamp[64][FFL_NSTAMP];
extern "C" int ffl_debug_read_stamps(unsigned long long *out) {
    return (int)hipMemcpyFromSymbol(out, HIP_SYMBOL(g_stamp), sizeof(unsigned long long) * 64 * FFL_NSTAMP);
}
#define FFL_DRAIN_MAX 8192
__device__ unsigned long long g_drain[3][FFL_DRAIN_MAX][2];
extern "C" int ffl_debug_read_drain(unsigned long long *out) {
    return (int)hipMemcpyFromSymbol(out, HIP_SYMBOL(g_drain), sizeof(unsigned long long) * 3 * FFL_DRAIN_MAX * 2);
}
#define FFL_DRAIN(e)                                                          \
    if (w >= 1024 && tid == 0 && blockIdx.x < FFL_DRAIN_MAX) g_drain[FIRST ? 0 : UPDATE ? 1 : 2][blockIdx.x][e] = wall_clock64();
#define FFL_T(i)                                                              \
    if (FFL_STAMP_ON && tid == 0) {                                           \
        const unsigned long long t_ = __builtin_readcyclecounter();          \
        sStamp[i] += t_ - sStamp[FFL_NSTAMP];                                 \
        sStamp[FFL_NSTAMP] = t_;                                              \
    }
#else
#define FFL_T(i)
#define FFL_DRAIN(e)
#endif


template <bool UPDATE, int FIRST>
__global__ __launch_bounds__(256, FIRST ? FFL_K5_WAVES_FIRST : FFL_K5_WAVES) void k_blur_solve(
    const float *__restrict__ Min, float *__restrict__ Mout, size_t M_stride, const float *__restrict__ R, size_t R_stride,
    size_t plane, const PairTab *__restrict__ pt, int level, int w, int h, BlurPlan plan, int pw, int ph, double usx, double usy,
    int store_flow, int order) {
    constexpr int TW = 64, TH = 16, LW = TW + 2 * FFL_WIN_R, LH = TH + 2 * FFL_WIN_R;
    constexpr int PX = 4;
    constexpr int NCARRY = LH - TH;
    constexpr int LW2 = 44;
    constexpr int GC = FIRST ? FFL_K5_GROUP_FIRST : FFL_K5_GROUP, NG = (5 + GC - 1) / GC;
    __shared__ double2 sS2[GC][TH][LW2];
    const int tid = threadIdx.x;
#ifdef FFL_STAMP
    __shared__ unsigned long long sStamp[FFL_NSTAMP + 1];
    const bool FFL_STAMP_ON = FIRST == 1 && w >= 1024;
    if (FFL_STAMP_ON && tid == 0) {
        for (int i = 0; i < FFL_NSTAMP; i++) sStamp[i] = 0;
        sStamp[FFL_NSTAMP] = __builtin_readcyclecounter();
    }
#endif
    int b, tile_x, row0, nrb;
    if (!ffl_blur_block(plan, blockIdx.x, (w + TW - 1) / TW, order, b, tile_x, row0, nrb)) return;
    FFL_DRAIN(0)
    const int x0 = tile_x * TW;
    const float *Mb = Min + (size_t)b * M_stride;

    const int q = __builtin_amdgcn_readfirstlane(tid >> 6);
    const int ty = (tid & 63) >> 2, kk = tid & 3;
    const int lx0 = 16 * kk + 4 * q;
    double *sS = reinterpret_cast<double *>(&sS2[0][0][0]);
    const int vcc = tid / LW, vtx = tid - vcc * LW;
    const int vgx = min(max(x0 + vtx - FFL_WIN_R, 0), w - 1);
    const unsigned pitch = (unsigned)w * 4u;
    float carry[NG][NCARRY];
    const double scale = 1.0 / (FFL_WIN * FFL_WIN);
    float2 *flow = reinterpret_cast<float2 *>(pt->flow[level][b]);
    const float *R0 = R + (size_t)pt->u0[b] * R_stride, *R1 = R + (size_t)pt->u1[b] * R_stride;
    float *Mo = Mout + (size_t)b * M_stride;
    constexpr int FP = TW + 2;
    float4 *sF4 = reinterpret_cast<float4 *>(&sS2[0][0][0]);
    constexpr int UP = 80;
    __shared__ float sM34[FIRST ? 5 - GC : 1][FIRST ? TH : 1][FIRST ? UP : 1];
    float *sM012 = reinterpret_cast<float *>(&sS2[0][0][0]);
    static_assert(GC * TH * UP * 4 <= (int)sizeof(sS2), "the first group's staged rows must fit the column sums");
    const float2 *prevf = reinterpret_cast<const float2 *>(pt->flow[min(level + 1, FFL_MAX_LEVELS - 1)][b]);
    struct UStageA {
        float a1, b1;
        float4 c0, c1;
        bool first0, first1;
        int r, tx, gx, gy;
    };
    const bool half_scale = usx == 0.5 && usy == 0.5;
    auto phase_u = [&](int y0, int jbase, int nrows) {
        const int N = LW * nrows;
        auto coords = [&](int i, int &r, int &tx, int &gx, int &gy) {
            r = i / LW;
            tx = i - r * LW;
            gy = min(max(y0 - FFL_WIN_R + jbase + r, 0), h - 1);
            gx = min(max(x0 + tx - FFL_WIN_R, 0), w - 1);
        };
        auto issue = [&](int i) {
            UStageA A;
            coords(i, A.r, A.tx, A.gx, A.gy);
            const int gx = A.gx, gy = A.gy;
            if (FIRST == 1) {
                int xa0, xa1, ya0, ya1;
                if (half_scale) {
                    ffl_resize_coord_half(gx, pw, xa0, xa1, A.a1);
                    ffl_resize_coord_half(gy, ph, ya0, ya1, A.b1);
                } else {
                    ffl_resize_coord(gx, pw, usx, xa0, xa1, A.a1);
                    ffl_resize_coord(gy, ph, usy, ya0, ya1, A.b1);
                }
                const float *pf = reinterpret_cast<const float *>(prevf);
                const unsigned r0o = (unsigned)ya0 * (unsigned)pw, r1o = (unsigned)ya1 * (unsigned)pw;
                const int xq = min(xa0, pw - 2);
                A.c0 = ffl_gload4(pf, 8u * (r0o + xq));
                A.c1 = ffl_gload4(pf, 8u * (r1o + xq));
                A.first0 = xa0 == xq;
                A.first1 = xa1 == xq;
            }
            return A;
        };
        int i = tid;
        if (i >= N) return;
        UStageA A = issue(i);
#pragma unroll 1
        for (;;) {
            const int r = A.r, tx = A.tx, gx = A.gx, gy = A.gy;
            const int inext = i + 256;
            const bool more = inext < N;
            float2 f = make_float2(0.f, 0.f);
            if (FIRST == 1) f = ffl_upsample2(A.c0, A.c1, A.first0, A.first1, A.a1, A.b1);
            float r0[5];
            {
                const unsigned o = (unsigned)gy * (unsigned)w + (unsigned)gx;
#pragma unroll
                for (int c = 0; c < 5; c++) r0[c] = *ffl_at<float>(R0 + c * plane, o);
            }
            const UmLoc L = ffl_um_locate(w, h, gx, gy, f.x, f.y);
            const unsigned o1 = L.inside ? (unsigned)L.y1 * (unsigned)w + (unsigned)L.x1 : 0u;
            ffl_f2u t[5], u[5];
#pragma unroll
            for (int c = 0; c < 5; c++) {
                t[c] = ffl_ld_corner(R1 + c * plane, o1);
                u[c] = ffl_ld_corner(R1 + c * plane, o1 + (unsigned)w);
            }
            const UStageA Anext = issue(more ? inext : i);
            float b[5];
#pragma unroll
            for (int c = 0; c < 5; c++) b[c] = L.a00 * t[c].x + L.a01 * t[c].y + L.a10 * u[c].x + L.a11 * u[c].y;
            float m[5];
            ffl_um_finish(r0, b, L.inside, w, h, gx, gy, f.x, f.y, m);
#pragma unroll
            for (int c = 0; c < GC; c++) sM012[(c * TH + r) * UP + tx] = m[c];
#pragma unroll
            for (int c = GC; c < 5; c++) sM34[c - GC][r][tx] = m[c];
            if (!more) break;
            A = Anext;
            i = inext;
        }
    };

#pragma unroll 1
    for (int rb = 0; rb < nrb; rb++) {
        const int y0 = (row0 + rb) * TH;
        if (y0 >= h) break;
        double acc[5][PX];
        if (FIRST) {
            if (rb == 0) {
                phase_u(y0, 0, NCARRY);
                __syncthreads();
#pragma unroll
                for (int g = 0; g < NG; g++) {
                    const int c0 = g * GC, nc = min(GC, 5 - c0);
                    if (tid < nc * LW) {
#pragma unroll
                        for (int j = 0; j < NCARRY; j++)
                            carry[g][j] = g == 0 ? sM012[(vcc * TH + j) * UP + vtx] : sM34[c0 - GC + vcc][j][vtx];
                    }
                }
                __syncthreads();
            }
            FFL_T(0)
            phase_u(y0, NCARRY, TH);
            FFL_T(1)
            __syncthreads();
            FFL_T(2)
        }
#pragma unroll
        for (int g = 0; g < NG; g++) {
            const int c0 = g * GC, nc = min(GC, 5 - c0);
            if (g) __syncthreads();
            FFL_T(3)
            const bool vlane = tid < nc * LW;
            float v[LH];
            if (vlane) {
                const char *Mbb = reinterpret_cast<const char *>(Mb);
                const unsigned lane_byte = ((unsigned)((c0 + vcc) * plane) + (unsigned)vgx) * 4u;
                if (FIRST) {
#pragma unroll
                    for (int j = 0; j < NCARRY; j++) v[j] = carry[g][j];
#pragma unroll
                    for (int j = 0; j < TH; j++)
                        v[NCARRY + j] = g == 0 ? sM012[(vcc * TH + j) * UP + vtx] : sM34[c0 - GC + vcc][j][vtx];
                } else {
                    if (rb == 0) {
#pragma unroll
                        for (int j = 0; j < NCARRY; j++) {
                            const unsigned gy = (unsigned)min(max(y0 + j - FFL_WIN_R, 0), h - 1);
                            v[j] = *reinterpret_cast<const float *>(Mbb + (gy * pitch + lane_byte));
                        }
                    } else {
#pragma unroll
                        for (int j = 0; j < NCARRY; j++) v[j] = carry[g][j];
                    }
#pragma unroll
                    for (int j = NCARRY; j < LH; j++) {
                        const unsigned gy = (unsigned)min(max(y0 + j - FFL_WIN_R, 0), h - 1);
                        v[j] = *reinterpret_cast<const float *>(Mbb + (gy * pitch + lane_byte));
                    }
                }
            }
            if (FIRST && g == 0) __syncthreads();
            if (vlane) {
#pragma unroll
                for (int j = 0; j < NCARRY; j++) carry[g][j] = v[TH + j];
                double o[TH];
                ffl_box_block16(v, o);
                const int pos = vtx + 2 * (vtx >> 4);
#pragma unroll
                for (int j = 0; j < TH; j++) sS[(vcc * TH + j) * (2 * LW2) + pos] = o[j];
            }
            FFL_T(4)
            __syncthreads();
            FFL_T(5)
#pragma unroll
            for (int cc = 0; cc < GC; cc++) {
                if (cc >= nc) break;
                double d[PX + 14];
                const double2 *src = &sS2[cc][ty][9 * kk];
#define FFL_K5_H(Q)                                                                        \
    {                                                                                      \
        _Pragma("unroll") for (int j = 0; j < (PX + 14) / 2; j++) {                        \
            const double2 t2 = src[2 * (Q) + j + ((4 * (Q) + 2 * j) >> 4)];                \
            d[2 * j] = t2.x;                                                               \
            d[2 * j + 1] = t2.y;                                                           \
        }                                                                                  \
        ffl_box_quarter<Q>(d, acc[c0 + cc]);                                               \
    }
                switch (q) {
                    case 0: FFL_K5_H(0) break;
                    case 1: FFL_K5_H(1) break;
                    case 2: FFL_K5_H(2) break;
                    default: FFL_K5_H(3) break;
                }
#undef FFL_K5_H
            }
        }

        FFL_T(6)
        __syncthreads();
        FFL_T(7)
        {
            float2 f[PX];
#pragma unroll
            for (int p = 0; p < PX; p++) {
                double g11 = acc[0][p] * scale, g12 = acc[1][p] * scale, g22 = acc[2][p] * scale,
                       h1 = acc[3][p] * scale, h2 = acc[4][p] * scale;
                double idet = 1.0 / (g11 * g22 - g12 * g12 + 1e-3);
                f[p].x = (float)((g11 * h2 - g12 * h1) * idet);
                f[p].y = (float)((g22 * h1 - g12 * h2) * idet);
            }
            sF4[(ty * FP + lx0) / 2] = make_float4(f[0].x, f[0].y, f[1].x, f[1].y);
            sF4[(ty * FP + lx0) / 2 + 1] = make_float4(f[2].x, f[2].y, f[3].x, f[3].y);
        }
        FFL_T(8)
        __syncthreads();
        FFL_T(9)
        if (UPDATE) {
            const int lx = tid & 63, x = min(x0 + lx, w - 1);
            const float2 *sF2 = reinterpret_cast<const float2 *>(sF4);
            ffl_um_rows<TH / 4>(R0, R1, Mo, plane, w, h, x, x0 + lx < w, y0 + (tid >> 6),
                                [&](int k) { return sF2[((tid >> 6) + 4 * k) * FP + lx]; },
                                [&](unsigned o, float2 d) {
                                    if (store_flow) *reinterpret_cast<float2 *>(ffl_at<float>(reinterpret_cast<float *>(flow), 2u * o)) = d;
                                });
        } else {
            const int lx = 2 * (tid & 31), x = x0 + lx;
            if (x < w) {
                const bool second = x + 1 < w;
#pragma unroll
                for (int k = 0; k < TH / 8; k++) {
                    const int ly = (tid >> 5) + 8 * k;
                    if (y0 + ly >= h) continue;
                    const float4 ff = sF4[(ly * FP + lx) >> 1];
                    const size_t o = (size_t)(y0 + ly) * w + x;
                    if (second) {
                        ffl_f4u t;
                        t.x = ff.x; t.y = ff.y; t.z = ff.z; t.w = ff.w;
                        *reinterpret_cast<ffl_f4u *>(flow + o) = t;
                    } else {
                        flow[o] = make_float2(ff.x, ff.y);
                    }
                }
            }
        }
        FFL_T(10)
        __syncthreads();
        FFL_T(11)
    }
#ifdef FFL_STAMP
    if (FFL_STAMP_ON && tid == 0)
        for (int i = 0; i < FFL_NSTAMP; i++) g_stamp[blockIdx.x & 63][i] = sStamp[i];
#endif
    FFL_DRAIN(1)
}

static int ffl_blur_rows_per_wg(int tiles_x, int tiles_y, int nB, int min_wgs) {
    if (nB > 32 && tiles_x * tiles_y >= 256) nB = 32;
    for (int s = 1; s <= tiles_y; s++) {
        const int nrb = (tiles_y + s - 1) / s;
        if (nrb > 64) continue;
        if ((long)tiles_x * ((tiles_y + nrb - 1) / nrb) * nB >= min_wgs || nrb == 1) return nrb;
    }
    return 1;
}

unsigned ffl_blur_plan(int tiles_x, int tiles_y, int nB, int slots, const FflOptions &opt, BlurPlan *plan) {
    const int nrb = opt.blur_rows > 0 ? opt.blur_rows : ffl_blur_rows_per_wg(tiles_x, tiles_y, nB, opt.blur_min_wgs);
    int P = opt.blur_taper_pairs;
    if (P == 0 && opt.blur_taper && nrb > 2 && slots > 0) {
        const long per_pair = (long)tiles_x * ((tiles_y + nrb - 1) / nrb);
        P = (int)std::min((slots + 2 * per_pair) / (4 * per_pair), (long)(nB / 4));
    }
    const int p2 = std::min(P, nB), p1 = std::min(P, nB - p2);
    const int pairs[FFL_BLUR_SEGS] = {nB - p1 - p2, p1, p2};
    const int rows[FFL_BLUR_SEGS] = {nrb, (nrb + 1) / 2, std::max(1, (nrb + 3) / 4)};
    *plan = BlurPlan{};
    unsigned grid = 0;
    int pair0 = 0;
    for (int i = 0; i < FFL_BLUR_SEGS; i++) {
        if (pairs[i] == 0) continue;
        const int strips = (tiles_y + rows[i] - 1) / rows[i];
        plan->s[plan->n++] = BlurSeg{(int)grid, pair0, pairs[i], rows[i], strips};
        grid += ffl_tile_grid(tiles_x, strips, pairs[i]);
        pair0 += pairs[i];
    }
    return grid;
}

template <typename K>
static int ffl_k5_slots(K k, int cus) {
    int per_cu = 0;
    if (hipOccupancyMaxActiveBlocksPerMultiprocessor(&per_cu, k, 256, 0) != hipSuccess) return 0;
    return per_cu * cus;
}
bool ffl_blur_slots(BlurSlots *out) {
    int dev = 0, cus = 0;
    if (hipGetDevice(&dev) != hipSuccess || hipDeviceGetAttribute(&cus, hipDeviceAttributeMultiprocessorCount, dev) != hipSuccess)
        return false;
    *out = BlurSlots{ffl_k5_slots(k_blur_solve<true, 1>, cus), ffl_k5_slots(k_blur_solve<true, 2>, cus),
                     ffl_k5_slots(k_blur_solve<true, 0>, cus), ffl_k5_slots(k_blur_solve<false, 0>, cus)};
    return out->first > 0 && out->first_zero > 0 && out->update > 0 && out->last > 0;
}
#ifdef FFL_STAMP
extern "C" int ffl_debug_blur_slots(int *out) {
    BlurSlots s;
    if (!ffl_blur_slots(&s)) return 1;
    out[0] = s.first; out[1] = s.first_zero; out[2] = s.update; out[3] = s.last;
    return 0;
}
#endif

template <typename K>
static void ffl_launch_k5(K k, const float *Min, float *Mout, size_t M_stride, const float *R, size_t R_stride, size_t plane,
                          const PairTab *pt, int level, int nB, int lw, int lh, int pw, int ph, int store_flow,
                          const FflOptions &opt, int slots, hipStream_t st) {
    BlurPlan plan;
    dim3 grid(ffl_blur_plan((lw + 63) / 64, (lh + 15) / 16, nB, slots, opt, &plan));
    hipLaunchKernelGGL(k, grid, dim3(256), 0, st, Min, Mout, M_stride, R, R_stride, plane, pt, level, lw, lh, plan, pw, ph,
                       pw > 0 ? (double)pw / lw : 1.0, pw > 0 ? (double)ph / lh : 1.0, store_flow, opt.tile_order);
}

void ffl_launch_blur_solve(const float *Min, float *Mout, size_t M_stride, const float *R, size_t R_stride,
                           size_t plane, const PairTab *pt, int level, int nB, int lw, int lh, int update, int store_flow,
                           const FflOptions &opt, const BlurSlots &slots, hipStream_t st) {
    ffl_launch_k5(update ? k_blur_solve<true, 0> : k_blur_solve<false, 0>, Min, Mout, M_stride, R, R_stride, plane, pt, level,
                  nB, lw, lh, 0, 0, update ? store_flow : 1, opt, update ? slots.update : slots.last, st);
}

void ffl_launch_blur_solve_first(float *Mout, size_t M_stride, const float *R, size_t R_stride, size_t plane,
                                 const PairTab *pt, int level, int nB, int lw, int lh, int pw, int ph, const FflOptions &opt,
                                 const BlurSlots &slots, hipStream_t st) {
    ffl_launch_k5(pw > 0 ? k_blur_solve<true, 1> : k_blur_solve<true, 2>, (const float *)nullptr, Mout, M_stride, R, R_stride,
                  plane, pt, level, nB, lw, lh, pw, ph, 0, opt, pw > 0 ? slots.first : slots.first_zero, st);
}
```

### include/ffl.h

```cpp
#ifndef FFL_H
#define FFL_H

#include <stddef.h>
#include <stdint.h>

#ifdef __cplusplus
extern "C" {
#endif

#define FFL_OK 0
#define FFL_ERR_INVALID 1
#define FFL_ERR_HIP 2
#define FFL_ERR_NO_DEVICE 3
#define FFL_ERR_STATE 4

#define FFL_MAX_BATCH 256

typedef struct ffl_ctx ffl_ctx;

int ffl_device_count(void);

int ffl_create(int device, int width, int height, int n_frame_slots, int n_flow_slots, int max_batch,
               ffl_ctx **out);
void ffl_destroy(ffl_ctx *ctx);
// ... 218 lines not shown
int ffl_texture_params_check(const ffl_texture_params *p);

int ffl_texture_weights(ffl_ctx *ctx, int n, const int *fslots, const ffl_texture_params *p, const ffl_dev_weights *gate,
                        const ffl_dev_weights *out, uint64_t stream);

#define FFL_MAX_CELLS 64
typedef struct ffl_cell_record {
    double mean_u, mean_v, mean_mag, var_mag;
} ffl_cell_record;
typedef struct ffl_grid_centre {
    double cx, cy, total_var;
    int32_t cells, empty;
} ffl_grid_centre;

int ffl_cell_grid_check(int width, int height, int cells, int *cell_w, int *cell_h);

int ffl_cell_stats(ffl_ctx *ctx, int n, const int *flow_slots, int cells, ffl_cell_record *cells_dev,
                   ffl_grid_centre *centres_dev, uint64_t stream);

int ffl_radial_window_axes_centres(ffl_ctx *ctx, int n_seq, const int *seq_slots, int first, int n, int radius,
                                   float cut_threshold, int pov_mode, const void *centres_dev, ptrdiff_t centre_stride_bytes,
                                   ffl_axes_record *out_dev, uint64_t stream);

int ffl_cells_extra_bytes(int width, int height, int cells, size_t *bytes);

enum { FFL_MAX_TRACKS = 8, FFL_MAX_TRACK_RADIUS = 32 };
enum { FFL_TRACK_HOLD = 0, FFL_TRACK_HOME = 1 };
enum { FFL_TRACK_OK = 0, FFL_TRACK_CUT = 1, FFL_TRACK_LOST = 2, FFL_TRACK_CLAMPED = 4 };
typedef struct ffl_track_params {
    int radius, on_cut;
    float cut_threshold;
} ffl_track_params;
typedef struct ffl_track_state {
    double x, y, home_x, home_y;
    int64_t steps;
    int32_t lost_run, pad;
} ffl_track_state;
typedef struct ffl_track_record {
    double x, y, du, dv, sw;
    int32_t count, status;
} ffl_track_record;
int ffl_track_default_params(ffl_track_params *out);
int ffl_track_params_check(const ffl_track_params *p);

int ffl_track_advance(ffl_ctx *ctx, int n, const int *seq_slots, int n_tracks, const ffl_track_params *p,
                      const ffl_dev_weights *weights, ffl_track_state *state_dev, ffl_track_record *out_dev, uint64_t stream);

typedef struct ffl_roi_params {
    float ax, ay;
    int soft;
} ffl_roi_params;
int ffl_roi_default_params(ffl_roi_params *out);
int ffl_roi_params_check(const ffl_roi_params *p);

int ffl_roi_weights(ffl_ctx *ctx, int n, const void *centres_dev, ptrdiff_t centre_stride_bytes, const ffl_roi_params *p,
                    const ffl_dev_weights *gate, const ffl_dev_weights *out, uint64_t stream);

int ffl_radial_window_axes_weighted_centres(ffl_ctx *ctx, int n_seq, const int *seq_slots, int first, int n, int radius,
                                            float cut_threshold, int pov_mode, const ffl_dev_weights *w,
                                            const void *centres_dev, ptrdiff_t centre_stride_bytes, ffl_axes_record *out_dev,
                                            uint64_t stream);

enum { FFL_MOTION_TRANSLATION = 0, FFL_MOTION_RIGID = 1, FFL_MOTION_SIMILARITY = 2, FFL_MOTION_AFFINE = 3 };
enum { FFL_MOTION_OK = 0, FFL_MOTION_EMPTY = 1, FFL_MOTION_DEGENERATE = 2 };
enum { FFL_MOTION_N_SUMS = 12 };
typedef struct ffl_motion_params {
    int model, iterations;
    float tau;
} ffl_motion_params;
typedef struct ffl_motion_record {
    double a0, a1, a2, b0, b1, b2;
    double sw;
    int32_t model, status;
} ffl_motion_record;

int ffl_motion_default_params(ffl_motion_params *out);
int ffl_motion_params_check(const ffl_motion_params *p);

int ffl_motion_solve(const double *sums, int model, ffl_motion_record *out);

int ffl_motion_extra_bytes(int width, int height, size_t *bytes);

int ffl_motion_fit(ffl_ctx *ctx, int n, const int *flow_slots, const ffl_motion_params *p, const ffl_dev_weights *weights,
                   const void *prior_dev, ptrdiff_t prior_stride_bytes, ffl_motion_record *models_dev, double *sums_dev,
                   uint64_t stream);

int ffl_motion_subtract(ffl_ctx *ctx, int n, const int *src_slots, const int *dst_slots, const void *models_dev,
                        ptrdiff_t model_stride_bytes, int pov_mode, uint64_t stream);

int ffl_download_flow(ffl_ctx *ctx, int flow_slot, float *dst);

int ffl_upload_flow(ffl_ctx *ctx, int flow_slot, const float *src, int pov_mode);

int ffl_submit_pair(ffl_ctx *ctx, int slot, const uint8_t *prev, const uint8_t *next, int width, int height,
                    int channels, ptrdiff_t stride_bytes, int pov_mode);

int ffl_sync(ffl_ctx *ctx);


typedef struct ffl_dis_params {
    int finest_scale, patch_size, patch_stride, grad_descent_iters, var_refine_iters;
    float vr_alpha, vr_gamma, vr_delta;
    int use_mean_norm, use_spatial_prop, stripes;
} ffl_dis_params;

int ffl_dis_default_params(ffl_dis_params *out);

int ffl_dis_geometry(int width, int height, const ffl_dis_params *p, int *coarsest, int *finest);

int ffl_flow_pairs_dis(ffl_ctx *ctx, int n, const int *fslot0, const int *fslot1, const int *flow_slots, int pov_mode,
                       const ffl_dis_params *p);

int ffl_debug_dis_pair(ffl_ctx *ctx, int f0, int f1, const ffl_dis_params *p, int scale, int stage, float *out);


typedef struct ffl_farneback_params {
    float pyr_scale;
    int levels;
    int winsize;
    int iterations;
    int poly_n;
    float poly_sigma;
    int flags;
} ffl_farneback_params;

int ffl_farneback_default_params(ffl_farneback_params *out);

int ffl_farneback_geometry(int width, int height, const ffl_farneback_params *p, int *n_scales, size_t *work_bytes_per_pair);

int ffl_farneback_extra_bytes(int width, int height, int max_batch, const ffl_farneback_params *p, size_t *bytes);

int ffl_flow_pairs_farneback(ffl_ctx *ctx, int n, const int *fslot0, const int *fslot1, const int *flow_slots, int pov_mode,
                             const ffl_farneback_params *p);

#define FFL_FB_USE_INITIAL_FLOW 4u
#define FFL_FB_GAUSSIAN_WINDOW  256u

int ffl_flow_pairs_farneback_ex(ffl_ctx *ctx, int n, const int *fslot0, const int *fslot1, const int *flow_slots,
                                int pov_mode, const ffl_farneback_params *p, unsigned mode);


int ffl_num_levels(const ffl_ctx *ctx);
int ffl_level_size(const ffl_ctx *ctx, int level, int *out_wh);

int ffl_download_frame(ffl_ctx *ctx, int fslot, uint8_t *dst);

int ffl_debug_pair(ffl_ctx *ctx, int f0, int f1, int level, int iter, float *I0, float *I1, float *R0, float *R1,
                   float *M, float *flow);

int ffl_debug_blur_plan(int tiles_x, int tiles_y, int n_pairs, int slots, int blur_rows, int blur_min_wgs, int blur_taper,
                        int blur_taper_pairs, int tile_order, int *segments, int *n_segments, int *grid, int *blocks,
                        int max_blocks);


int ffl_set_option(const char *name, int value);
int ffl_ctx_set_option(ffl_ctx *ctx, const char *name, int value);
int ffl_ctx_get_option(ffl_ctx *ctx, const char *name, int *value);

int ffl_graph_stats(ffl_ctx *ctx, int *captured, int *replayed, int *capture_failures);

int ffl_profile_enable(ffl_ctx *ctx, unsigned class_mask);
#define FFL_PROFILE_ALL 0xFFu
#define FFL_K_GRAY 0
#define FFL_K_PYRAMID 1
#define FFL_K_POLYEXP 2
#define FFL_K_FRONTEND 3
#define FFL_K_UPDATE_MATRICES 4
#define FFL_K_BLUR_SOLVE 5
#define FFL_K_PASS1 6
#define FFL_K_RADIAL 7
#define FFL_K_COUNT 8
int ffl_profile_read(ffl_ctx *ctx, int kernel_class, int *launches, double *total_ms);
const char *ffl_kernel_name(int kernel_class);

#ifdef __cplusplus
}
#endif
#endif
```

Before: 6577.

## Fuse coarse pyramid levels' blur-solve iterations into one per-pair kernel

```diff
diff --git a/funscript_flow_amd/_capi.py b/funscript_flow_amd/_capi.py
--- a/funscript_flow_amd/_capi.py
+++ b/funscript_flow_amd/_capi.py
@@ -781,6 +781,7 @@
     "ffl_download_frame": (_i, (_ctx, _i, _vp)),
     "ffl_debug_pair": (_i, (_ctx,) + (_i,) * 4 + (_vp,) * 6),
     "ffl_debug_blur_plan": (_i, (_i,) * 9 + (_ip, _ip, _ip, _ip, _i)),
+    "ffl_debug_coarse_run": (_i, (_i, _i, _ip, _ip, _ip)),
     "ffl_set_option": (_i, (_str, _i)),
     "ffl_ctx_set_option": (_i, (_ctx, _str, _i)),
     "ffl_ctx_get_option": (_i, (_ctx, _str, _ip)),
@@ -843,6 +844,12 @@
     out = np.zeros((grid.value, 4), np.int32)
     _check(L.ffl_debug_blur_plan(*args, seg, C.byref(n), C.byref(grid), out.ctypes.data_as(_ip), grid.value), exc=ValueError)
     return segments, grid.value, out
+
+
+def coarse_run(width, height):
+    levels, n_run, sizes = C.c_int(), C.c_int(), (C.c_int * 16)()
+    _check(load().ffl_debug_coarse_run(int(width), int(height), C.byref(levels), sizes, C.byref(n_run)), exc=ValueError)
+    return [(sizes[2 * k], sizes[2 * k + 1]) for k in range(levels.value + 1)], n_run.value
 
 
 def device_count():
diff --git a/funscript_flow_amd/csrc/blur_solve_body.inc b/funscript_flow_amd/csrc/blur_solve_body.inc
--- /dev/null
+++ b/funscript_flow_amd/csrc/blur_solve_body.inc
@@ -0,0 +1,261 @@
+    constexpr int TW = G::TW, TH = G::TH, LW = G::LW, LH = G::LH;
+    constexpr int PX = 4;
+    constexpr int NCARRY = LH - TH;
+    constexpr int LW2 = G::LW2;
+    constexpr int GC = G::GC, NG = G::NG;
+    FFL_DRAIN(0)
+    const int x0 = tile_x * TW;
+    const float *Mb = Min + (size_t)b * M_stride;
+
+    const int q = __builtin_amdgcn_readfirstlane(tid >> 6);
+    const int ty = (tid & 63) >> 2, kk = tid & 3;
+    const int lx0 = 16 * kk + 4 * q;
+    double *sS = reinterpret_cast<double *>(&sS2[0][0][0]);
+    const int vcc = tid / LW, vtx = tid - vcc * LW;
+    const int vgx = min(max(x0 + vtx - FFL_WIN_R, 0), w - 1);
+    const unsigned pitch = (unsigned)w * 4u;
+    float carry[NG][NCARRY];
+    const double scale = 1.0 / (FFL_WIN * FFL_WIN);
+    float2 *flow = reinterpret_cast<float2 *>(pt->flow[level][b]);
+    const float *R0 = R + (size_t)pt->u0[b] * R_stride, *R1 = R + (size_t)pt->u1[b] * R_stride;
+    float *Mo = Mout + (size_t)b * M_stride;
+    constexpr int FP = TW + 2;
+    float4 *sF4 = reinterpret_cast<float4 *>(&sS2[0][0][0]);
+    constexpr int UP = G::UP;
+#ifndef FFL_BLUR_BODY_LDS_GIVEN
+    __shared__ float sM34[FIRST ? 5 - GC : 1][FIRST ? TH : 1][FIRST ? UP : 1];
+#endif
+    float *sM012 = reinterpret_cast<float *>(&sS2[0][0][0]);
+    static_assert(GC * TH * UP * 4 <= G::S2_COUNT * 16, "the first group's staged rows must fit the column sums");
+    const float2 *prevf = reinterpret_cast<const float2 *>(pt->flow[min(level + 1, FFL_MAX_LEVELS - 1)][b]);
+    struct UStageA {
+        float a1, b1;
+        float4 c0, c1;
+        bool first0, first1;
+        int r, tx, gx, gy;
+    };
+    const bool half_scale = usx == 0.5 && usy == 0.5;
+    auto phase_u = [&](int y0, int jbase, int nrows) {
+        const int N = LW * nrows;
+        auto coords = [&](int i, int &r, int &tx, int &gx, int &gy) {
+            r = i / LW;
+            tx = i - r * LW;
+            gy = min(max(y0 - FFL_WIN_R + jbase + r, 0), h - 1);
+            gx = min(max(x0 + tx - FFL_WIN_R, 0), w - 1);
+        };
+        auto issue = [&](int i) {
+            UStageA A;
+            coords(i, A.r, A.tx, A.gx, A.gy);
+            const int gx = A.gx, gy = A.gy;
+            if (FIRST == 1) {
+                int xa0, xa1, ya0, ya1;
+                if (half_scale) {
+                    ffl_resize_coord_half(gx, pw, xa0, xa1, A.a1);
+                    ffl_resize_coord_half(gy, ph, ya0, ya1, A.b1);
+                } else {
+                    ffl_resize_coord(gx, pw, usx, xa0, xa1, A.a1);
+                    ffl_resize_coord(gy, ph, usy, ya0, ya1, A.b1);
+                }
+                const float *pf = reinterpret_cast<const float *>(prevf);
+                const unsigned r0o = (unsigned)ya0 * (unsigned)pw, r1o = (unsigned)ya1 * (unsigned)pw;
+                const int xq = min(xa0, pw - 2);
+                A.c0 = ffl_gload4(pf, 8u * (r0o + xq));
+                A.c1 = ffl_gload4(pf, 8u * (r1o + xq));
+                A.first0 = xa0 == xq;
+                A.first1 = xa1 == xq;
+            }
+            return A;
+        };
+        int i = tid;
+        if (i >= N) return;
+        UStageA A = issue(i);
+#pragma unroll 1
+        for (;;) {
+            const int r = A.r, tx = A.tx, gx = A.gx, gy = A.gy;
+            const int inext = i + 256;
+            const bool more = inext < N;
+            float2 f = make_float2(0.f, 0.f);
+            if (FIRST == 1) f = ffl_upsample2(A.c0, A.c1, A.first0, A.first1, A.a1, A.b1);
+            float r0[5];
+            {
+                const unsigned o = (unsigned)gy * (unsigned)w + (unsigned)gx;
+#pragma unroll
+                for (int c = 0; c < 5; c++) r0[c] = *ffl_at<float>(R0 + c * plane, o);
+            }
+            const UmLoc L = ffl_um_locate(w, h, gx, gy, f.x, f.y);
+            const unsigned o1 = L.inside ? (unsigned)L.y1 * (unsigned)w + (unsigned)L.x1 : 0u;
+            ffl_f2u t[5], u[5];
+#pragma unroll
+            for (int c = 0; c < 5; c++) {
+                t[c] = ffl_ld_corner(R1 + c * plane, o1);
+                u[c] = ffl_ld_corner(R1 + c * plane, o1 + (unsigned)w);
+            }
+            const UStageA Anext = issue(more ? inext : i);
+            float b[5];
+#pragma unroll
+            for (int c = 0; c < 5; c++) b[c] = L.a00 * t[c].x + L.a01 * t[c].y + L.a10 * u[c].x + L.a11 * u[c].y;
+            float m[5];
+            ffl_um_finish(r0, b, L.inside, w, h, gx, gy, f.x, f.y, m);
+#pragma unroll
+            for (int c = 0; c < GC; c++) sM012[(c * TH + r) * UP + tx] = m[c];
+#pragma unroll
+            for (int c = GC; c < 5; c++) sM34[c - GC][r][tx] = m[c];
+            if (!more) break;
+            A = Anext;
+            i = inext;
+        }
+    };
+
+#pragma unroll 1
+    for (int rb = 0; rb < nrb; rb++) {
+        const int y0 = (row0 + rb) * TH;
+        if (y0 >= h) break;
+        double acc[5][PX];
+        if (FIRST) {
+            if (rb == 0) {
+                phase_u(y0, 0, NCARRY);
+                __syncthreads();
+#pragma unroll
+                for (int g = 0; g < NG; g++) {
+                    const int c0 = g * GC, nc = min(GC, 5 - c0);
+                    if (tid < nc * LW) {
+#pragma unroll
+                        for (int j = 0; j < NCARRY; j++)
+                            carry[g][j] = g == 0 ? sM012[(vcc * TH + j) * UP + vtx] : sM34[c0 - GC + vcc][j][vtx];
+                    }
+                }
+                __syncthreads();
+            }
+            FFL_T(0)
+            phase_u(y0, NCARRY, TH);
+            FFL_T(1)
+            __syncthreads();
+            FFL_T(2)
+        }
+#pragma unroll
+        for (int g = 0; g < NG; g++) {
+            const int c0 = g * GC, nc = min(GC, 5 - c0);
+            if (g) __syncthreads();
+            FFL_T(3)
+            const bool vlane = tid < nc * LW;
+            float v[LH];
+            if (vlane) {
+                const char *Mbb = reinterpret_cast<const char *>(Mb);
+                const unsigned lane_byte = ((unsigned)((c0 + vcc) * plane) + (unsigned)vgx) * 4u;
+                if (FIRST) {
+#pragma unroll
+                    for (int j = 0; j < NCARRY; j++) v[j] = carry[g][j];
+#pragma unroll
+                    for (int j = 0; j < TH; j++)
+                        v[NCARRY + j] = g == 0 ? sM012[(vcc * TH + j) * UP + vtx] : sM34[c0 - GC + vcc][j][vtx];
+                } else {
+                    if (rb == 0) {
+#pragma unroll
+                        for (int j = 0; j < NCARRY; j++) {
+                            const unsigned gy = (unsigned)min(max(y0 + j - FFL_WIN_R, 0), h - 1);
+                            v[j] = *reinterpret_cast<const float *>(Mbb + (gy * pitch + lane_byte));
+                        }
+                    } else {
+#pragma unroll
+                        for (int j = 0; j < NCARRY; j++) v[j] = carry[g][j];
+                    }
+#pragma unroll
+                    for (int j = NCARRY; j < LH; j++) {
+                        const unsigned gy = (unsigned)min(max(y0 + j - FFL_WIN_R, 0), h - 1);
+                        v[j] = *reinterpret_cast<const float *>(Mbb + (gy * pitch + lane_byte));
+                    }
+                }
+            }
+            if (FIRST && g == 0) __syncthreads();
+            if (vlane) {
+#pragma unroll
+                for (int j = 0; j < NCARRY; j++) carry[g][j] = v[TH + j];
+                double o[TH];
+                ffl_box_block16(v, o);
+                const int pos = vtx + 2 * (vtx >> 4);
+#pragma unroll
+                for (int j = 0; j < TH; j++) sS[(vcc * TH + j) * (2 * LW2) + pos] = o[j];
+            }
+            FFL_T(4)
+            __syncthreads();
+            FFL_T(5)
+#pragma unroll
+            for (int cc = 0; cc < GC; cc++) {
+                if (cc >= nc) break;
+                double d[PX + 14];
+                const double2 *src = &sS2[cc][ty][9 * kk];
+#define FFL_K5_H(Q)                                                                        \
+    {                                                                                      \
+        _Pragma("unroll") for (int j = 0; j < (PX + 14) / 2; j++) {                        \
+            const double2 t2 = src[2 * (Q) + j + ((4 * (Q) + 2 * j) >> 4)];                \
+            d[2 * j] = t2.x;                                                               \
+            d[2 * j + 1] = t2.y;                                                           \
+        }                                                                                  \
+        ffl_box_quarter<Q>(d, acc[c0 + cc]);                                               \
+    }
+                switch (q) {
+                    case 0: FFL_K5_H(0) break;
+                    case 1: FFL_K5_H(1) break;
+                    case 2: FFL_K5_H(2) break;
+                    default: FFL_K5_H(3) break;
+                }
+#undef FFL_K5_H
+            }
+        }
+
+        FFL_T(6)
+        __syncthreads();
+        FFL_T(7)
+        {
+            float2 f[PX];
+#pragma unroll
+            for (int p = 0; p < PX; p++) {
+                double g11 = acc[0][p] * scale, g12 = acc[1][p] * scale, g22 = acc[2][p] * scale,
+                       h1 = acc[3][p] * scale, h2 = acc[4][p] * scale;
+                double idet = 1.0 / (g11 * g22 - g12 * g12 + 1e-3);
+                f[p].x = (float)((g11 * h2 - g12 * h1) * idet);
+                f[p].y = (float)((g22 * h1 - g12 * h2) * idet);
+            }
+            sF4[(ty * FP + lx0) / 2] = make_float4(f[0].x, f[0].y, f[1].x, f[1].y);
+            sF4[(ty * FP + lx0) / 2 + 1] = make_float4(f[2].x, f[2].y, f[3].x, f[3].y);
+        }
+        FFL_T(8)
+        __syncthreads();
+        FFL_T(9)
+        if (UPDATE) {
+            const int lx = tid & 63, x = min(x0 + lx, w - 1);
+            const float2 *sF2 = reinterpret_cast<const float2 *>(sF4);
+            ffl_um_rows<TH / 4>(R0, R1, Mo, plane, w, h, x, x0 + lx < w, y0 + (tid >> 6),
+                                [&](int k) { return sF2[((tid >> 6) + 4 * k) * FP + lx]; },
+                                [&](unsigned o, float2 d) {
+                                    if (store_flow) *reinterpret_cast<float2 *>(ffl_at<float>(reinterpret_cast<float *>(flow), 2u * o)) = d;
+                                });
+        } else {
+            const int lx = 2 * (tid & 31), x = x0 + lx;
+            if (x < w) {
+                const bool second = x + 1 < w;
+#pragma unroll
+                for (int k = 0; k < TH / 8; k++) {
+                    const int ly = (tid >> 5) + 8 * k;
+                    if (y0 + ly >= h) continue;
+                    const float4 ff = sF4[(ly * FP + lx) >> 1];
+                    const size_t o = (size_t)(y0 + ly) * w + x;
+                    if (second) {
+                        ffl_f4u t;
+                        t.x = ff.x; t.y = ff.y; t.z = ff.z; t.w = ff.w;
+                        *reinterpret_cast<ffl_f4u *>(flow + o) = t;
+                    } else {
+                        flow[o] = make_float2(ff.x, ff.y);
+                    }
+                }
+            }
+        }
+        FFL_T(10)
+        __syncthreads();
+        FFL_T(11)
+    }
+#ifdef FFL_STAMP
+    if (FFL_STAMP_ON && tid == 0)
+        for (int i = 0; i < FFL_NSTAMP; i++) g_stamp[blockIdx.x & 63][i] = sStamp[i];
+#endif
+    FFL_DRAIN(1)
diff --git a/funscript_flow_amd/csrc/ffl_api.hip b/funscript_flow_amd/csrc/ffl_api.hip
--- a/funscript_flow_amd/csrc/ffl_api.hip
+++ b/funscript_flow_amd/csrc/ffl_api.hip
@@ -438,6 +438,12 @@
     }
 }
 
+static int coarse_run(const Geometry &geo) {
+    int lw[8];
+    for (int k = 0; k <= geo.levels; k++) lw[k] = geo.lv[k].lw;
+    return ffl_coarse_run(lw, geo.levels);
+}
+
 #define FFL_FRAME_SIZE_RULE "unsupported frame size %dx%d (16x16 .. 20*w*h < 2^32)"
 static bool frame_size_ok(int w, int h) { return !(w < 16 || h < 16 || (long)w * h * 20 >= (1L << 32)); }
 static bool counts_ok(int n_frame_slots, int n_flow_slots, int max_batch) {
@@ -1305,7 +1311,23 @@
     }
 
     int pw = 0, ph = 0;
-    for (int k = c->geo.levels; k >= 0; k--) {
+    int k_top = c->geo.levels;
+    if (const int nrun = coarse_run(c->geo); nrun > 0 && !cap && c->opt.fuse_first > 0 && c->opt.coarse_pair && n >= c->opt.coarse_pair_min) {
+        CoarseRun run = {};
+        for (; run.n < nrun; k_top--) {
+            const LevelGeom &g = c->geo.lv[k_top];
+            run.lv[run.n++] = CoarseLevel{k_top, g.lw, g.lh, pw, ph, pw > 0 ? (double)pw / g.lw : 1.0, pw > 0 ? (double)ph / g.lh : 1.0,
+                                          {L.d_M[0], L.d_M[1]}, 0, L.d_R + c->lay.r_off[k_top], pt};
+            pw = g.lw;
+            ph = g.lh;
+        }
+        run.agent = c->opt.coarse_pair == 2;
+        for (int i = 0; i < run.n; i++)
+            run.lv[i].m_stride = 5 * (size_t)run.lv[run.n - 1].w * run.lv[run.n - 1].h;
+        ProfScope ps(c, FFL_K_BLUR_SOLVE, st);
+        ffl_launch_coarse_pair(run, n, st);
+    }
+    for (int k = k_top; k >= 0; k--) {
         const LevelGeom &g = c->geo.lv[k];
         const int lw = g.lw, lh = g.lh;
         const size_t plane = (size_t)lw * lh;
@@ -3376,6 +3398,20 @@
     return FFL_OK;
 }
 
+int ffl_debug_coarse_run(int width, int height, int *levels, int *sizes, int *n_run) {
+    if (!frame_size_ok(width, height) || !levels || !sizes || !n_run)
+        return set_err(nullptr, FFL_ERR_INVALID, "ffl_debug_coarse_run: " FFL_FRAME_SIZE_RULE " or NULL output", width, height);
+    LevelRule r;
+    level_rule(width, height, 0.5, 3, &r);
+    *levels = r.levels;
+    for (int k = 0; k <= r.levels; k++) {
+        sizes[2 * k] = r.lw[k];
+        sizes[2 * k + 1] = r.lh[k];
+    }
+    *n_run = ffl_coarse_run(r.lw, r.levels);
+    return FFL_OK;
+}
+
 int ffl_set_option(const char *name, int value) {
     if (!name) return FFL_ERR_INVALID;
     std::lock_guard<std::mutex> g(g_opt_mu);
diff --git a/funscript_flow_amd/csrc/ffl_kernels.h b/funscript_flow_amd/csrc/ffl_kernels.h
--- a/funscript_flow_amd/csrc/ffl_kernels.h
+++ b/funscript_flow_amd/csrc/ffl_kernels.h
@@ -133,6 +133,8 @@
     int pyr_coarse = 1;
     int fuse_l0_blur = 1;
     int fb_general = 0;
+    int coarse_pair = 1;
+    int coarse_pair_min = 160;
 };
 struct FflOptionRow {
     const char *name;
@@ -153,6 +155,8 @@
     {"pyr_coarse", &FflOptions::pyr_coarse, INT_MIN, INT_MAX, true},
     {"fuse_l0_blur", &FflOptions::fuse_l0_blur, INT_MIN, INT_MAX, true},
     {"fb_general", &FflOptions::fb_general, 0, 1, false},
+    {"coarse_pair", &FflOptions::coarse_pair, 0, 2, false},
+    {"coarse_pair_min", &FflOptions::coarse_pair_min, 1, FFL_MAXB + 1, false},
 };
 
 #define FFL_BLUR_SEGS 3
@@ -166,6 +170,25 @@
 struct BlurSlots {
     int first, first_zero, update, last;
 };
+
+struct CoarseLevel {
+    int level, w, h, pw, ph;
+    double usx, usy;
+    float *M[2];
+    size_t m_stride;
+    const float *R;
+    const PairTab *pt;
+};
+struct CoarseRun {
+    CoarseLevel lv[FFL_MAX_LEVELS];
+    int n;
+    int agent;
+};
+inline int ffl_coarse_run(const int *lw, int levels) {
+    int n = 0;
+    while (n <= levels && n < 2 && (lw[levels - n] + 63) / 64 == 1) n++;
+    return n;
+}
 
 bool ffl_launch_pyr_multi(const uint8_t *gray_base, size_t gray_stride, const UTab *ut, int nU, const PyrJob *levels, int n,
                           const FflOptions &opt, hipStream_t st);
@@ -197,6 +220,7 @@
 void ffl_launch_blur_solve_first(float *Mout, size_t M_stride, const float *R, size_t R_stride, size_t plane,
                                  const PairTab *pt, int level, int nB, int lw, int lh, int pw, int ph, const FflOptions &opt,
                                  const BlurSlots &slots, hipStream_t st);
+void ffl_launch_coarse_pair(const CoarseRun &run, int nB, hipStream_t st);
 bool ffl_blur_slots(BlurSlots *out);
 unsigned ffl_blur_plan(int tiles_x, int tiles_y, int nB, int slots, const FflOptions &opt, BlurPlan *plan);
 
diff --git a/funscript_flow_amd/csrc/kernels_farneback.hip b/funscript_flow_amd/csrc/kernels_farneback.hip
--- a/funscript_flow_amd/csrc/kernels_farneback.hip
+++ b/funscript_flow_amd/csrc/kernels_farneback.hip
@@ -959,17 +959,23 @@
 #endif
 
 
+template <int FIRST>
+struct BlurGeom {
+    static constexpr int TW = 64, TH = 16, LW = TW + 2 * FFL_WIN_R, LH = TH + 2 * FFL_WIN_R;
+    static constexpr int LW2 = 44;
+    static constexpr int GC = FIRST ? FFL_K5_GROUP_FIRST : FFL_K5_GROUP, NG = (5 + GC - 1) / GC;
+    static constexpr int UP = 80;
+    static constexpr int S2_COUNT = GC * TH * LW2, M34_COUNT = FIRST ? (5 - GC) * TH * UP : 1;
+    static constexpr int ARENA_BYTES = S2_COUNT * 16 + (FIRST ? M34_COUNT * 4 : 0);
+};
+
 template <bool UPDATE, int FIRST>
 __global__ __launch_bounds__(256, FIRST ? FFL_K5_WAVES_FIRST : FFL_K5_WAVES) void k_blur_solve(
     const float *__restrict__ Min, float *__restrict__ Mout, size_t M_stride, const float *__restrict__ R, size_t R_stride,
     size_t plane, const PairTab *__restrict__ pt, int level, int w, int h, BlurPlan plan, int pw, int ph, double usx, double usy,
     int store_flow, int order) {
-    constexpr int TW = 64, TH = 16, LW = TW + 2 * FFL_WIN_R, LH = TH + 2 * FFL_WIN_R;
-    constexpr int PX = 4;
-    constexpr int NCARRY = LH - TH;
-    constexpr int LW2 = 44;
-    constexpr int GC = FIRST ? FFL_K5_GROUP_FIRST : FFL_K5_GROUP, NG = (5 + GC - 1) / GC;
-    __shared__ double2 sS2[GC][TH][LW2];
+    using G = BlurGeom<FIRST>;
+    __shared__ double2 sS2[G::GC][G::TH][G::LW2];
     const int tid = threadIdx.x;
 #ifdef FFL_STAMP
     __shared__ unsigned long long sStamp[FFL_NSTAMP + 1];
@@ -980,261 +986,8 @@
     }
 #endif
     int b, tile_x, row0, nrb;
-    if (!ffl_blur_block(plan, blockIdx.x, (w + TW - 1) / TW, order, b, tile_x, row0, nrb)) return;
-    FFL_DRAIN(0)
-    const int x0 = tile_x * TW;
-    const float *Mb = Min + (size_t)b * M_stride;
-
-    const int q = __builtin_amdgcn_readfirstlane(tid >> 6);
-    const int ty = (tid & 63) >> 2, kk = tid & 3;
-    const int lx0 = 16 * kk + 4 * q;
-    double *sS = reinterpret_cast<double *>(&sS2[0][0][0]);
-    const int vcc = tid / LW, vtx = tid - vcc * LW;
-    const int vgx = min(max(x0 + vtx - FFL_WIN_R, 0), w - 1);
-    const unsigned pitch = (unsigned)w * 4u;
-    float carry[NG][NCARRY];
-    const double scale = 1.0 / (FFL_WIN * FFL_WIN);
-    float2 *flow = reinterpret_cast<float2 *>(pt->flow[level][b]);
-    const float *R0 = R + (size_t)pt->u0[b] * R_stride, *R1 = R + (size_t)pt->u1[b] * R_stride;
-    float *Mo = Mout + (size_t)b * M_stride;
-    constexpr int FP = TW + 2;
-    float4 *sF4 = reinterpret_cast<float4 *>(&sS2[0][0][0]);
-    constexpr int UP = 80;
-    __shared__ float sM34[FIRST ? 5 - GC : 1][FIRST ? TH : 1][FIRST ? UP : 1];
-    float *sM012 = reinterpret_cast<float *>(&sS2[0][0][0]);
-    static_assert(GC * TH * UP * 4 <= (int)sizeof(sS2), "the first group's staged rows must fit the column sums");
-    const float2 *prevf = reinterpret_cast<const float2 *>(pt->flow[min(level + 1, FFL_MAX_LEVELS - 1)][b]);
-    struct UStageA {
-        float a1, b1;
-        float4 c0, c1;
-        bool first0, first1;
-        int r, tx, gx, gy;
-    };
-    const bool half_scale = usx == 0.5 && usy == 0.5;
-    auto phase_u = [&](int y0, int jbase, int nrows) {
-        const int N = LW * nrows;
-        auto coords = [&](int i, int &r, int &tx, int &gx, int &gy) {
-            r = i / LW;
-            tx = i - r * LW;
-            gy = min(max(y0 - FFL_WIN_R + jbase + r, 0), h - 1);
-            gx = min(max(x0 + tx - FFL_WIN_R, 0), w - 1);
-        };
-        auto issue = [&](int i) {
-            UStageA A;
-            coords(i, A.r, A.tx, A.gx, A.gy);
-            const int gx = A.gx, gy = A.gy;
-            if (FIRST == 1) {
-                int xa0, xa1, ya0, ya1;
-                if (half_scale) {
-                    ffl_resize_coord_half(gx, pw, xa0, xa1, A.a1);
-                    ffl_resize_coord_half(gy, ph, ya0, ya1, A.b1);
-                } else {
-                    ffl_resize_coord(gx, pw, usx, xa0, xa1, A.a1);
-                    ffl_resize_coord(gy, ph, usy, ya0, ya1, A.b1);
-                }
-                const float *pf = reinterpret_cast<const float *>(prevf);
-                const unsigned r0o = (unsigned)ya0 * (unsigned)pw, r1o = (unsigned)ya1 * (unsigned)pw;
-                const int xq = min(xa0, pw - 2);
-                A.c0 = ffl_gload4(pf, 8u * (r0o + xq));
-                A.c1 = ffl_gload4(pf, 8u * (r1o + xq));
-                A.first0 = xa0 == xq;
-                A.first1 = xa1 == xq;
-            }
-            return A;
-        };
-        int i = tid;
-        if (i >= N) return;
-        UStageA A = issue(i);
-#pragma unroll 1
-        for (;;) {
-            const int r = A.r, tx = A.tx, gx = A.gx, gy = A.gy;
-            const int inext = i + 256;
-            const bool more = inext < N;
-            float2 f = make_float2(0.f, 0.f);
-            if (FIRST == 1) f = ffl_upsample2(A.c0, A.c1, A.first0, A.first1, A.a1, A.b1);
-            float r0[5];
-            {
-                const unsigned o = (unsigned)gy * (unsigned)w + (unsigned)gx;
-#pragma unroll
-                for (int c = 0; c < 5; c++) r0[c] = *ffl_at<float>(R0 + c * plane, o);
-            }
-            const UmLoc L = ffl_um_locate(w, h, gx, gy, f.x, f.y);
-            const unsigned o1 = L.inside ? (unsigned)L.y1 * (unsigned)w + (unsigned)L.x1 : 0u;
-            ffl_f2u t[5], u[5];
-#pragma unroll
-            for (int c = 0; c < 5; c++) {
-                t[c] = ffl_ld_corner(R1 + c * plane, o1);
-                u[c] = ffl_ld_corner(R1 + c * plane, o1 + (unsigned)w);
-            }
-            const UStageA Anext = issue(more ? inext : i);
-            float b[5];
-#pragma unroll
-            for (int c = 0; c < 5; c++) b[c] = L.a00 * t[c].x + L.a01 * t[c].y + L.a10 * u[c].x + L.a11 * u[c].y;
-            float m[5];
-            ffl_um_finish(r0, b, L.inside, w, h, gx, gy, f.x, f.y, m);
-#pragma unroll
-            for (int c = 0; c < GC; c++) sM012[(c * TH + r) * UP + tx] = m[c];
-#pragma unroll
-            for (int c = GC; c < 5; c++) sM34[c - GC][r][tx] = m[c];
-            if (!more) break;
-            A = Anext;
-            i = inext;
-        }
-    };
-
-#pragma unroll 1
-    for (int rb = 0; rb < nrb; rb++) {
-        const int y0 = (row0 + rb) * TH;
-        if (y0 >= h) break;
-        double acc[5][PX];
-        if (FIRST) {
-            if (rb == 0) {
-                phase_u(y0, 0, NCARRY);
-                __syncthreads();
-#pragma unroll
-                for (int g = 0; g < NG; g++) {
-                    const int c0 = g * GC, nc = min(GC, 5 - c0);
-                    if (tid < nc * LW) {
-#pragma unroll
-                        for (int j = 0; j < NCARRY; j++)
-                            carry[g][j] = g == 0 ? sM012[(vcc * TH + j) * UP + vtx] : sM34[c0 - GC + vcc][j][vtx];
-                    }
-                }
-                __syncthreads();
-            }
-            FFL_T(0)
-            phase_u(y0, NCARRY, TH);
-            FFL_T(1)
-            __syncthreads();
-            FFL_T(2)
-        }
-#pragma unroll
-        for (int g = 0; g < NG; g++) {
-            const int c0 = g * GC, nc = min(GC, 5 - c0);
-            if (g) __syncthreads();
-            FFL_T(3)
-            const bool vlane = tid < nc * LW;
-            float v[LH];
-            if (vlane) {
-                const char *Mbb = reinterpret_cast<const char *>(Mb);
-                const unsigned lane_byte = ((unsigned)((c0 + vcc) * plane) + (unsigned)vgx) * 4u;
-                if (FIRST) {
-#pragma unroll
-                    for (int j = 0; j < NCARRY; j++) v[j] = carry[g][j];
-#pragma unroll
-                    for (int j = 0; j < TH; j++)
-                        v[NCARRY + j] = g == 0 ? sM012[(vcc * TH + j) * UP + vtx] : sM34[c0 - GC + vcc][j][vtx];
-                } else {
-                    if (rb == 0) {
-#pragma unroll
-                        for (int j = 0; j < NCARRY; j++) {
-                            const unsigned gy = (unsigned)min(max(y0 + j - FFL_WIN_R, 0), h - 1);
-                            v[j] = *reinterpret_cast<const float *>(Mbb + (gy * pitch + lane_byte));
-                        }
-                    } else {
-#pragma unroll
-                        for (int j = 0; j < NCARRY; j++) v[j] = carry[g][j];
-                    }
-#pragma unroll
-                    for (int j = NCARRY; j < LH; j++) {
-                        const unsigned gy = (unsigned)min(max(y0 + j - FFL_WIN_R, 0), h - 1);
-                        v[j] = *reinterpret_cast<const float *>(Mbb + (gy * pitch + lane_byte));
-                    }
-                }
-            }
-            if (FIRST && g == 0) __syncthreads();
-            if (vlane) {
-#pragma unroll
-                for (int j = 0; j < NCARRY; j++) carry[g][j] = v[TH + j];
-                double o[TH];
-                ffl_box_block16(v, o);
-                const int pos = vtx + 2 * (vtx >> 4);
-#pragma unroll
-                for (int j = 0; j < TH; j++) sS[(vcc * TH + j) * (2 * LW2) + pos] = o[j];
-            }
-            FFL_T(4)
-            __syncthreads();
-            FFL_T(5)
-#pragma unroll
-            for (int cc = 0; cc < GC; cc++) {
-                if (cc >= nc) break;
-                double d[PX + 14];
-                const double2 *src = &sS2[cc][ty][9 * kk];
-#define FFL_K5_H(Q)                                                                        \
-    {                                                                                      \
-        _Pragma("unroll") for (int j = 0; j < (PX + 14) / 2; j++) {                        \
-            const double2 t2 = src[2 * (Q) + j + ((4 * (Q) + 2 * j) >> 4)];                \
-            d[2 * j] = t2.x;                                                               \
-            d[2 * j + 1] = t2.y;                                                           \
-        }                                                                                  \
-        ffl_box_quarter<Q>(d, acc[c0 + cc]);                                               \
-    }
-                switch (q) {
-                    case 0: FFL_K5_H(0) break;
-                    case 1: FFL_K5_H(1) break;
-                    case 2: FFL_K5_H(2) break;
-                    default: FFL_K5_H(3) break;
-                }
-#undef FFL_K5_H
-            }
-        }
-
-        FFL_T(6)
-        __syncthreads();
-        FFL_T(7)
-        {
-            float2 f[PX];
-#pragma unroll
-            for (int p = 0; p < PX; p++) {
-                double g11 = acc[0][p] * scale, g12 = acc[1][p] * scale, g22 = acc[2][p] * scale,
-                       h1 = acc[3][p] * scale, h2 = acc[4][p] * scale;
-                double idet = 1.0 / (g11 * g22 - g12 * g12 + 1e-3);
-                f[p].x = (float)((g11 * h2 - g12 * h1) * idet);
-                f[p].y = (float)((g22 * h1 - g12 * h2) * idet);
-            }
-            sF4[(ty * FP + lx0) / 2] = make_float4(f[0].x, f[0].y, f[1].x, f[1].y);
-            sF4[(ty * FP + lx0) / 2 + 1] = make_float4(f[2].x, f[2].y, f[3].x, f[3].y);
-        }
-        FFL_T(8)
-        __syncthreads();
-        FFL_T(9)
-        if (UPDATE) {
-            const int lx = tid & 63, x = min(x0 + lx, w - 1);
-            const float2 *sF2 = reinterpret_cast<const float2 *>(sF4);
-            ffl_um_rows<TH / 4>(R0, R1, Mo, plane, w, h, x, x0 + lx < w, y0 + (tid >> 6),
-                                [&](int k) { return sF2[((tid >> 6) + 4 * k) * FP + lx]; },
-                                [&](unsigned o, float2 d) {
-                                    if (store_flow) *reinterpret_cast<float2 *>(ffl_at<float>(reinterpret_cast<float *>(flow), 2u * o)) = d;
-                                });
-        } else {
-            const int lx = 2 * (tid & 31), x = x0 + lx;
-            if (x < w) {
-                const bool second = x + 1 < w;
-#pragma unroll
-                for (int k = 0; k < TH / 8; k++) {
-                    const int ly = (tid >> 5) + 8 * k;
-                    if (y0 + ly >= h) continue;
-                    const float4 ff = sF4[(ly * FP + lx) >> 1];
-                    const size_t o = (size_t)(y0 + ly) * w + x;
-                    if (second) {
-                        ffl_f4u t;
-                        t.x = ff.x; t.y = ff.y; t.z = ff.z; t.w = ff.w;
-                        *reinterpret_cast<ffl_f4u *>(flow + o) = t;
-                    } else {
-                        flow[o] = make_float2(ff.x, ff.y);
-                    }
-                }
-            }
-        }
-        FFL_T(10)
-        __syncthreads();
-        FFL_T(11)
-    }
-#ifdef FFL_STAMP
-    if (FFL_STAMP_ON && tid == 0)
-        for (int i = 0; i < FFL_NSTAMP; i++) g_stamp[blockIdx.x & 63][i] = sStamp[i];
-#endif
-    FFL_DRAIN(1)
+    if (!ffl_blur_block(plan, blockIdx.x, (w + G::TW - 1) / G::TW, order, b, tile_x, row0, nrb)) return;
+#include "blur_solve_body.inc"
 }
 
 static int ffl_blur_rows_per_wg(int tiles_x, int tiles_y, int nB, int min_wgs) {
@@ -1316,3 +1069,59 @@
     ffl_launch_k5(pw > 0 ? k_blur_solve<true, 1> : k_blur_solve<true, 2>, (const float *)nullptr, Mout, M_stride, R, R_stride,
                   plane, pt, level, nB, lw, lh, pw, ph, 0, opt, pw > 0 ? slots.first : slots.first_zero, st);
 }
+
+template <bool UPDATE, int FIRST, int IN, int OUT>
+__device__ __forceinline__ void ffl_coarse_step(const CoarseRun &run, int i, double2 *arena) {
+    asm volatile("" : "+s"(i));
+    const CoarseLevel &lv = run.lv[i];
+    using G = BlurGeom<FIRST>;
+    double2 (&sS2)[G::GC][G::TH][G::LW2] = *reinterpret_cast<double2 (*)[G::GC][G::TH][G::LW2]>(arena);
+    float (&sM34)[FIRST ? 5 - G::GC : 1][FIRST ? G::TH : 1][FIRST ? G::UP : 1] =
+        *reinterpret_cast<float (*)[FIRST ? 5 - G::GC : 1][FIRST ? G::TH : 1][FIRST ? G::UP : 1]>(arena + G::S2_COUNT);
+#ifdef FFL_STAMP
+    unsigned long long *sStamp = nullptr;
+    const bool FFL_STAMP_ON = false;
+#endif
+    const int tid = threadIdx.x;
+    const float *Min = IN < 0 ? nullptr : lv.M[IN < 0 ? 0 : IN];
+    float *Mout = lv.M[OUT];
+    const float *R = lv.R;
+    const PairTab *pt = lv.pt;
+    const size_t plane = (size_t)lv.w * lv.h, M_stride = lv.m_stride, R_stride = 5 * plane;
+    const int level = lv.level, w = lv.w, h = lv.h, pw = FIRST == 1 ? lv.pw : 0, ph = FIRST == 1 ? lv.ph : 0;
+    const double usx = FIRST == 1 ? lv.usx : 1.0, usy = FIRST == 1 ? lv.usy : 1.0;
+    const int store_flow = UPDATE ? 0 : 1;
+    const int b = blockIdx.x, tile_x = 0, row0 = 0, nrb = (h + G::TH - 1) / G::TH;
+#define FFL_BLUR_BODY_LDS_GIVEN
+#include "blur_solve_body.inc"
+#undef FFL_BLUR_BODY_LDS_GIVEN
+}
+
+__global__ __launch_bounds__(256, 2) void k_coarse_pair(CoarseRun run) {
+    constexpr int ARENA = BlurGeom<1>::ARENA_BYTES;
+    static_assert(ARENA >= BlurGeom<0>::ARENA_BYTES && ARENA == BlurGeom<2>::ARENA_BYTES, "the arena is the largest body's");
+    static_assert(ARENA <= 45 * 1024 && BlurGeom<1>::S2_COUNT == BlurGeom<0>::S2_COUNT, "three workgroups per CU");
+    __shared__ double2 arena[ARENA / 16];
+    auto handoff = [&]() {
+        __syncthreads();
+        if (run.agent) {
+            __threadfence();
+            asm volatile("s_waitcnt vmcnt(0)" ::: "memory");
+            __syncthreads();
+        }
+    };
+#pragma unroll 1
+    for (int i = 0; i < run.n; i++) {
+        if (i) handoff();
+        if (run.lv[i].pw > 0) ffl_coarse_step<true, 1, -1, 1>(run, i, arena);
+        else ffl_coarse_step<true, 2, -1, 1>(run, i, arena);
+        handoff();
+        ffl_coarse_step<true, 0, 1, 0>(run, i, arena);
+        handoff();
+        ffl_coarse_step<false, 0, 0, 1>(run, i, arena);
+    }
+}
+
+void ffl_launch_coarse_pair(const CoarseRun &run, int nB, hipStream_t st) {
+    hipLaunchKernelGGL(k_coarse_pair, dim3(nB), dim3(256), 0, st, run);
+}
diff --git a/include/ffl.h b/include/ffl.h
--- a/include/ffl.h
+++ b/include/ffl.h
@@ -394,6 +394,8 @@
                         int blur_taper_pairs, int tile_order, int *segments, int *n_segments, int *grid, int *blocks,
                         int max_blocks);
 
+int ffl_debug_coarse_run(int width, int height, int *levels, int *sizes, int *n_run);
+
 
 int ffl_set_option(const char *name, int value);
 int ffl_ctx_set_option(ffl_ctx *ctx, const char *name, int value);
```

After: 6436. 2.2% lower.
